# COMP6248-Reproducability-Challenge/selfsupervised-denoising

Hardware: AMD Instinct MI355X
Metric: training patches/sec (64x64 gauss25 SSDN) (higher is better)
Workload: dtype f16

## Files before the change

include/ssdn_hip.h:

```cpp
#ifndef SSDN_HIP_H
#define SSDN_HIP_H

#include <stdint.h>

#ifdef __cplusplus
extern "C" {
#endif
#if defined(__GNUC__) || defined(__clang__)
#pragma GCC visibility push(default)
#endif

#define SSDN_ABI_VERSION 19
#define SSDN_MAX_TAPS 9

typedef struct ssdn_view {
    void* p;
    int32_t cs;
    int32_t co;
} ssdn_view;

enum ssdn_op_type {
    SSDN_OP_PACK_INPUT = 1,
    SSDN_OP_CONV = 2,
    SSDN_OP_POOL_FWD = 3,
    SSDN_OP_POOL_BWD = 4,
    SSDN_OP_UPSUM_BWD = 5,
    SSDN_OP_UNROT_FWD = 6,
    SSDN_OP_UNROT_BWD = 7,
    SSDN_OP_WGRAD = 8,
    SSDN_OP_WREDUCE = 9,
    SSDN_OP_WPACK = 10,
    SSDN_OP_GRAD_PACK = 11,
    SSDN_OP_HEAD_SSDN = 12,
    SSDN_OP_HEAD_FINAL = 13,
    SSDN_OP_SPATIAL_MEAN = 14,
    SSDN_OP_MSE = 15,
    SSDN_OP_MASK_MSE = 16,
    SSDN_OP_ADAM = 17,
    SSDN_OP_METRICS = 18,
    SSDN_OP_ZERO = 19,
    SSDN_OP_EVENT_RECORD = 20,
    SSDN_OP_NOISE = 21,
    SSDN_OP_INPUT_GRAD = 22,
    SSDN_OP_HEAD_VJP = 23,
    SSDN_OP_MSE_VJP = 24,
    SSDN_OP_ACCUM = 25
};

typedef struct ssdn_op {
    int32_t type;
    int32_t lane;
    const void* args;
} ssdn_op;

typedef struct ssdn_pack_input_args {
    const float* src;
    ssdn_view dst;
    int32_t B, C, H, W;
    int32_t R;
    int32_t cpad;
} ssdn_pack_input_args;

typedef struct ssdn_conv_args {
    ssdn_view src0;
    ssdn_view src1;
    int32_t c0, c1, up0;
    int32_t N, H, W;
    int32_t ntaps;
    int32_t dy[SSDN_MAX_TAPS];
    int32_t dx[SSDN_MAX_TAPS];
    const void* w;
    int32_t M, Mpad, Ktot;
    const float* bias;
    int32_t act;
    ssdn_view mask;
    ssdn_view add;
    ssdn_view dst;
    float* dst32;
    int32_t ltw, lth, ltn;
    int32_t kc;
    int32_t bf16;
    const void* wc;
    int32_t kreal;
    ssdn_view pool;
    int32_t pool_shifted;
    ssdn_view upsum;
    ssdn_view upsum_mask;
    int32_t upsum_c;
    ssdn_view unrot;
    ssdn_view unrot_mask;
    const void* unrot_smask;
    ssdn_view urot;
    void* urot_smask;
    void* sign_out;
    const void* mask_sign;
    const void* upsum_mask_sign;
} ssdn_conv_args;

typedef struct ssdn_pool_args {
    ssdn_view act;
    ssdn_view pooled;
    ssdn_view dpool;
    ssdn_view dz;
    int32_t N, H, W, C;
    int32_t shifted;
    void* route;
} ssdn_pool_args;

typedef struct ssdn_upsum_args {
    ssdn_view src;
    ssdn_view mask;
    ssdn_view dst;
    int32_t N, H, W, C;
} ssdn_upsum_args;

typedef struct ssdn_unrot_args {
    ssdn_view src;
    ssdn_view dst;
    ssdn_view mask;
    int32_t B, P, C;
    void* smask;
} ssdn_unrot_args;

typedef struct ssdn_wgrad_args {
    ssdn_view dz;
    ssdn_view src0;
    ssdn_view src1;
    int32_t c0, c1, up0;
    int32_t N, H, W;
    int32_t ntaps;
    int32_t dy[SSDN_MAX_TAPS];
    int32_t dx[SSDN_MAX_TAPS];
    int32_t coff[SSDN_MAX_TAPS];
    int32_t M, Mpad, Ktot, Kpad;
    float* slab;
    float* bslab;
    int32_t nslabs;
    int32_t ltw, lth, ltn;
    int32_t csplit;
    int32_t mblocks;
    int32_t kreal;
    int32_t mega;
    float cost;
} ssdn_wgrad_args;

typedef struct ssdn_wreduce_args {
    const float* slab;
    const float* bslab;
    int32_t nslabs, ntaps, M, Mpad, Kpad;
    int32_t cin;
    int32_t cin_full;
    int32_t m_off, c_off;
    int32_t tapblock;
    float* gw;
    float* gb;
    const float* inv_scale;
    int32_t accumulate;
} ssdn_wreduce_args;

typedef struct ssdn_wpack_args {
    const float* w;
    void* wf;
    void* wd;
    int32_t M, cin, ntaps;
    int32_t c0, c1_real;
    int32_t Mpad_f, Ktot;
    int32_t Mpad_d, Kd;
    void* wfc;
    void* wdc;
} ssdn_wpack_args;

typedef struct ssdn_grad_pack_args {
    const float* g;
    ssdn_view dst;
    int32_t N, C, H, W, cpad;
    const uint32_t* gmax;
    float* scale_out;
} ssdn_grad_pack_args;

typedef struct ssdn_head_args {
    const float* net_out;
    const float* noisy;
    const float* noise_param;
    const float* est_raw;
    int32_t B, C, H, W;
    int32_t style, mode;
    int32_t want_grad;
    float* mu;
    float* pme;
    float* model_std;
    float* noise_std;
    float* g_net_out;
    float* partial;
    int32_t nchunks;
    uint32_t* gmax;
    int32_t diag;
} ssdn_head_args;

typedef struct ssdn_head_final_args {
    const float* partial;
    int32_t B, nchunks, H, W;
    int32_t mode;
    float* loss;
    float* g_est;
    float* g_sigma_out;
    uint32_t* gmax2;
} ssdn_head_final_args;

typedef struct ssdn_spatial_mean_args {
    const float* src;
    float* dst;
    int32_t B, HW;
} ssdn_spatial_mean_args;

typedef struct ssdn_mse_args {
    const float* out;
    const float* ref;
    const int64_t* coords;
    int32_t ncoords;
    int32_t B, C, H, W;
    float* loss;
    float* g;
    uint32_t* gmax;
} ssdn_mse_args;

typedef struct ssdn_head_vjp_args {
    const float* net_out;
    const float* noisy;
    const float* noise_param;
    const float* est_raw;
    int32_t B, C, H, W;
    int32_t style, mode;
    const float* w;
    const float* g_pme;
    const float* g_mu;
    int32_t keep;
    int32_t nchunks;
    float* g_net_out;
    float* partial;
    uint32_t* gmax;
    float* g_est;
    float* g_sigma_out;
    uint32_t* gmax2;
    float* g_noisy;
    int32_t diag;
} ssdn_head_vjp_args;

typedef struct ssdn_mse_vjp_args {
    const float* out;
    const float* ref;
    const int64_t* coords;
    int32_t ncoords;
    int32_t masked;
    int32_t B, C, H, W;
    int32_t keep;
    const float* w;
    const float* g_pme;
    float* g;
    uint32_t* gmax;
} ssdn_mse_vjp_args;

typedef struct ssdn_adam_args {
    float* p;
    const float* g;
    float* m;
    float* v;
    int64_t n;
    float lr, b1, b2, eps, bc1, bc2;
    float gscale;
} ssdn_adam_args;

typedef struct ssdn_metrics_args {
    const float* out;
    const float* mu;
    const float* clean;
    const float* loss;
    const float* model_std;
    const float* noise_std;
    const int32_t* ext;
    int32_t B, C, H, W;
    int32_t noise_n;
    float* per;
    float* acc;
} ssdn_metrics_args;

typedef struct ssdn_zero_args {
    void* p;
    int64_t bytes;
} ssdn_zero_args;

typedef struct ssdn_accum_args {
    float* dst;
    const float* src;
    int64_t n;
} ssdn_accum_args;

typedef struct ssdn_event_args {
    void* event;
} ssdn_event_args;

typedef struct ssdn_noise_args {
    const void* clean_u8;
    float* clean32;
    float* noisy32;
    float* ref32;
    float* param;
    float* param_ref;
    int64_t* coords;
    int32_t B, C, H, W;
    int32_t style;
    int32_t clip;
    float p_lo, p_hi;
    int32_t n2v_box;
    int32_t n2v_radius;
    uint64_t seed, offset;
} ssdn_noise_args;

typedef struct ssdn_input_grad_args {
    ssdn_view g_e0;
    ssdn_view g_d1a;
    const float* w_e;
    const float* w_d;
    float* out;
    int32_t B, C, H, W;
    int32_t R;
    int32_t ntaps;
    int32_t dy[SSDN_MAX_TAPS], dx[SSDN_MAX_TAPS];
    const float* add;
} ssdn_input_grad_args;

int ssdn_run_ops(const ssdn_op* ops, int n, void* stream);

int ssdn_stream_order(void* first, void* then);

int ssdn_conv_lds_bytes(const ssdn_conv_args* a);
int ssdn_wgrad_lds_bytes(const ssdn_wgrad_args* a);
int ssdn_wgrad_mega_ok(const ssdn_wgrad_args* a);
int ssdn_wgrad_variant(const ssdn_wgrad_args* a, int32_t* out9);

int ssdn_struct_size(int op_type);
int ssdn_abi_version(void);
const char* ssdn_last_error(void);
int ssdn_device_cus(void);

#define SSDN_PROF_CONV_MT3 0
#define SSDN_PROF_CONV_MT2 1
#define SSDN_PROF_CONV_MT1 2
#define SSDN_PROF_WGRAD 3
#define SSDN_PROF_GEMM 4
#define SSDN_PROF_CDMA_MT3 5
#define SSDN_PROF_CDMA_MT21 6
#define SSDN_PROF_WGRAD_SIDE 7
#define SSDN_PROF_KINDS 8
int ssdn_profile_enable(int kind, int max_launches);
int ssdn_profile_set_stride(int kind, int stride);
int ssdn_profile_read(int kind, double* total_ms, long long* launches, double* flops, double* bytes);

int ssdn_conv_set_mode(int mode);
int ssdn_conv_fuses_pool(const ssdn_conv_args* a);
int ssdn_conv_fuses_upsum(const ssdn_conv_args* a);
int ssdn_conv_fuses_unrot(const ssdn_conv_args* a);
int ssdn_conv_fuses_urot(const ssdn_conv_args* a);
int ssdn_conv_signs(const ssdn_conv_args* a);

int ssdn_chain_len(const ssdn_op* ops, int n);
int ssdn_conv_set_chain(int on);

int ssdn_wgrad_mergeable(const ssdn_wgrad_args* a);

#define SSDN_PLAN_REPACK 0
#define SSDN_PLAN_FORWARD 1
#define SSDN_PLAN_BACKWARD 2
#define SSDN_PLAN_OPTIMISER 3
#define SSDN_PLAN_PHASES 4
typedef struct ssdn_plan ssdn_plan;
int ssdn_plan_load(const void* blob, int64_t nbytes, ssdn_plan** out);
void ssdn_plan_destroy(ssdn_plan* plan);
int64_t ssdn_plan_arena_bytes(const ssdn_plan* plan);
const char* ssdn_plan_meta(const ssdn_plan* plan);
int ssdn_plan_bind(ssdn_plan* plan, void* arena);
int ssdn_plan_tensor(const ssdn_plan* plan, const char* name, void** ptr, int64_t* bytes);
int ssdn_plan_run(ssdn_plan* plan, int phase, void* stream);
int ssdn_plan_set_lr(ssdn_plan* plan, float lr, int step, float gscale);
int ssdn_net_forward(ssdn_plan* plan, void* stream);
int ssdn_train_step(ssdn_plan* plan, float lr, int step, void* stream);

void ssdn_debug_set_trace(void* device_buffer);
void* ssdn_debug_get_trace(void);

int ssdn_probe_mfma(const void* a_frag, const void* b_frag, float* d_out, void* stream);
int ssdn_probe_tr16(const void* lds_image, int image_bytes, const int32_t* lane_addr, void* out, void* stream);

#if defined(__GNUC__) || defined(__clang__)
#pragma GCC visibility pop
#endif
#ifdef __cplusplus
}
#endif
#endif
```

selfsupervised-denoising_amd/csrc/api.hip:

```cpp
#include "common.h"
#include <cstdarg>
#include <cstdio>
#include <cstdlib>

static thread_local char g_err[512] = "";
thread_local hipEvent_t g_ssdn_stop_event = nullptr;
thread_local bool g_ssdn_stop_used = false;
thread_local hipEvent_t g_ssdn_prof_start = nullptr, g_ssdn_prof_stop = nullptr;
thread_local bool g_ssdn_prof_used = false;

int ssdn_set_error(const char* fmt, ...) {
    va_list ap;
    va_start(ap, fmt);
    vsnprintf(g_err, sizeof(g_err), fmt, ap);
    va_end(ap);
    return -1;
}

#include <vector>
struct ProfSlot {
    bool on = false;
    std::vector<hipEvent_t> ev;
    size_t used = 0;
    double flops = 0.0, bytes = 0.0;
    long long seen = 0;
    int stride = 1;
    bool armed = false;
    bool attached = false;
};
static bool prof_single_launch(int id) { return id == SSDN_PROF_CDMA_MT3 || id == SSDN_PROF_CDMA_MT21 || id == SSDN_PROF_GEMM; }
static ProfSlot g_prof[SSDN_PROF_KINDS];

void prof_begin(int id, hipStream_t s) {
    ProfSlot& p = g_prof[id];
    p.armed = false;
    if (!p.on) return;
    const bool pick = p.seen++ % p.stride == 0;
    if (!pick || p.used + 2 > p.ev.size()) return;
    p.armed = true;
    p.attached = prof_single_launch(id) && !g_ssdn_stop_event;
    if (p.attached) {
        g_ssdn_prof_start = p.ev[p.used];
        g_ssdn_prof_stop = p.ev[p.used + 1];
        g_ssdn_prof_used = false;
    } else (void)hipEventRecord(p.ev[p.used], s);
}
void prof_end(int id, hipStream_t s, double flops, double bytes) {
    ProfSlot& p = g_prof[id];
    if (!p.on || !p.armed) return;
    p.armed = false;
    if (p.attached) {
        const bool used = g_ssdn_prof_used;
        g_ssdn_prof_start = g_ssdn_prof_stop = nullptr;
        g_ssdn_prof_used = false;
        if (!used) return;
    } else (void)hipEventRecord(p.ev[p.used + 1], s);
    p.used += 2;
    p.flops += flops;
    p.bytes += bytes;
}

__global__ void k_zero(uint4* p, long long n16) {
    long long i = (long long)blockIdx.x * blockDim.x + threadIdx.x;
    for (; i < n16; i += (long long)gridDim.x * blockDim.x) p[i] = make_uint4(0, 0, 0, 0);
}

extern "C" {

int ssdn_abi_version(void) { return SSDN_ABI_VERSION; }
const char* ssdn_last_error(void) { return g_err; }

int ssdn_device_cus(void) {
    int dev = 0, cus = 0;
    if (hipGetDevice(&dev) != hipSuccess) return ssdn_set_error("hipGetDevice failed");
    if (hipDeviceGetAttribute(&cus, hipDeviceAttributeMultiprocessorCount, dev) != hipSuccess)
        return ssdn_set_error("hipDeviceGetAttribute failed");
    return cus;
}

int ssdn_struct_size(int op_type) {
    switch (op_type) {
        case 0: return (int)sizeof(ssdn_op);
        case SSDN_OP_PACK_INPUT: return (int)sizeof(ssdn_pack_input_args);
        case SSDN_OP_CONV: return (int)sizeof(ssdn_conv_args);
        case SSDN_OP_POOL_FWD: case SSDN_OP_POOL_BWD: return (int)sizeof(ssdn_pool_args);
        case SSDN_OP_UPSUM_BWD: return (int)sizeof(ssdn_upsum_args);
        case SSDN_OP_UNROT_FWD: case SSDN_OP_UNROT_BWD: return (int)sizeof(ssdn_unrot_args);
        case SSDN_OP_WGRAD: return (int)sizeof(ssdn_wgrad_args);
        case SSDN_OP_WREDUCE: return (int)sizeof(ssdn_wreduce_args);
        case SSDN_OP_WPACK: return (int)sizeof(ssdn_wpack_args);
        case SSDN_OP_GRAD_PACK: return (int)sizeof(ssdn_grad_pack_args);
        case SSDN_OP_HEAD_SSDN: return (int)sizeof(ssdn_head_args);
        case SSDN_OP_HEAD_FINAL: return (int)sizeof(ssdn_head_final_args);
        case SSDN_OP_SPATIAL_MEAN: return (int)sizeof(ssdn_spatial_mean_args);
        case SSDN_OP_MSE: case SSDN_OP_MASK_MSE: return (int)sizeof(ssdn_mse_args);
        case SSDN_OP_ADAM: return (int)sizeof(ssdn_adam_args);
        case SSDN_OP_METRICS: return (int)sizeof(ssdn_metrics_args);
        case SSDN_OP_ZERO: return (int)sizeof(ssdn_zero_args);
        case SSDN_OP_EVENT_RECORD: return (int)sizeof(ssdn_event_args);
        case SSDN_OP_NOISE: return (int)sizeof(ssdn_noise_args);
        case SSDN_OP_INPUT_GRAD: return (int)sizeof(ssdn_input_grad_args);
        case SSDN_OP_HEAD_VJP: return (int)sizeof(ssdn_head_vjp_args);
        case SSDN_OP_MSE_VJP: return (int)sizeof(ssdn_mse_vjp_args);
        case SSDN_OP_ACCUM: return (int)sizeof(ssdn_accum_args);
        default: return -1;
    }
}

int ssdn_profile_enable(int kind, int max_launches) {
    if (kind < 0 || kind >= SSDN_PROF_KINDS) return ssdn_set_error("profile: bad kernel kind %d", kind);
    ProfSlot& p = g_prof[kind];
    for (hipEvent_t e : p.ev) (void)hipEventDestroy(e);
    p.ev.clear();
    p.used = 0;
    p.flops = p.bytes = 0.0;
    p.on = max_launches > 0;
    p.seen = 0;
    p.armed = false;
    for (int i = 0; i < 2 * max_launches; ++i) {
        hipEvent_t e;
        if (hipEventCreate(&e) != hipSuccess) return ssdn_set_error("profile: hipEventCreate failed");
        p.ev.push_back(e);
    }
    return 0;
}

int ssdn_profile_set_stride(int kind, int stride) {
    if (kind < 0 || kind >= SSDN_PROF_KINDS) return ssdn_set_error("profile: bad kernel kind %d", kind);
    if (stride < 1) return ssdn_set_error("profile: stride must be >= 1");
    g_prof[kind].stride = stride;
    return 0;
}

int ssdn_profile_read(int kind, double* total_ms, long long* launches, double* flops, double* bytes) {
    if (kind < 0 || kind >= SSDN_PROF_KINDS) return ssdn_set_error("profile: bad kernel kind %d", kind);
    ProfSlot& p = g_prof[kind];
    double ms = 0.0;
    for (size_t i = 0; i + 1 < p.used; i += 2) {
        if (hipEventSynchronize(p.ev[i + 1]) != hipSuccess) return ssdn_set_error("profile: hipEventSynchronize failed");
        float t = 0.f;
        if (hipEventElapsedTime(&t, p.ev[i], p.ev[i + 1]) != hipSuccess) return ssdn_set_error("profile: hipEventElapsedTime failed");
        ms += t;
    }
    *total_ms = ms;
    *launches = (long long)(p.used / 2);
    *flops = p.flops;
    *bytes = p.bytes;
    p.used = 0;
    p.flops = p.bytes = 0.0;
    return 0;
}

int ssdn_conv_lds_bytes(const ssdn_conv_args* a) { return conv_lds_bytes(a); }
int ssdn_wgrad_lds_bytes(const ssdn_wgrad_args* a) { return wgrad_lds_bytes(a); }
int ssdn_wgrad_mergeable(const ssdn_wgrad_args* a) { return a && wgrad_mergeable(a) ? 1 : 0; }
int ssdn_wgrad_mega_ok(const ssdn_wgrad_args* a) { return wgrad_mega_ok(a); }
int ssdn_conv_fuses_pool(const ssdn_conv_args* a) { return a && conv_fuses_pool(a) ? 1 : 0; }
int ssdn_conv_fuses_upsum(const ssdn_conv_args* a) { return a && conv_fuses_upsum(a) ? 1 : 0; }
int ssdn_conv_fuses_unrot(const ssdn_conv_args* a) { return a && conv_fuses_unrot(a) ? 1 : 0; }
int ssdn_conv_fuses_urot(const ssdn_conv_args* a) { return a && conv_fuses_urot(a) ? 1 : 0; }
int ssdn_conv_signs(const ssdn_conv_args* a) { return a && conv_signs(a) ? 1 : 0; }

#define SSDN_NEVENTS 256
#define SSDN_NLANES 4
#define SSDN_MAX_DEVICES 16
struct LaneSet {
    hipStream_t side[SSDN_NLANES] = {nullptr, nullptr, nullptr, nullptr};
    hipEvent_t ev[SSDN_NEVENTS];
    int ev_next = 0;
    bool ready = false;
};
static LaneSet g_lanesets[SSDN_MAX_DEVICES];
static LaneSet* lanes_get() {
    int dev = 0;
    if (hipGetDevice(&dev) != hipSuccess || dev < 0 || dev >= SSDN_MAX_DEVICES) { ssdn_set_error("lanes: bad current device"); return nullptr; }
    LaneSet& L = g_lanesets[dev];
    if (L.ready) return &L;
    for (int l = 1; l < SSDN_NLANES; ++l)
        if (hipStreamCreateWithFlags(&L.side[l], hipStreamNonBlocking) != hipSuccess) { ssdn_set_error("lanes: hipStreamCreate failed"); return nullptr; }
    for (int i = 0; i < SSDN_NEVENTS; ++i)
        if (hipEventCreateWithFlags(&L.ev[i], hipEventDisableTiming) != hipSuccess) { ssdn_set_error("lanes: hipEventCreate failed"); return nullptr; }
    L.ready = true;
    return &L;
}
static const unsigned g_lane_deps[SSDN_NLANES] = {0u, 1u << 0, (1u << 0) | (1u << 1) | (1u << 3), 1u << 0};

int ssdn_stream_order(void* first, void* then) {
    LaneSet* LS = lanes_get();
    if (!LS) return -1;
    hipEvent_t e = LS->ev[LS->ev_next++ % SSDN_NEVENTS];
    SSDN_CHECK_HIP(hipEventRecord(e, (hipStream_t)first));
    SSDN_CHECK_HIP(hipStreamWaitEvent((hipStream_t)then, e, 0));
    return 0;
}

int ssdn_run_ops(const ssdn_op* ops, int n, void* stream) {
    hipStream_t lane_s[SSDN_NLANES] = {(hipStream_t)stream, nullptr, nullptr, nullptr};
    g_ssdn_stop_event = nullptr;
    bool dirty[SSDN_NLANES][SSDN_NLANES] = {}, used[SSDN_NLANES] = {true, false, false, false};
    for (int d = 1; d < SSDN_NLANES; ++d) dirty[0][d] = true;
    static const bool one_lane = ssdn_tuning_env("SSDN_ONE_LANE") != nullptr;
    LaneSet* LS = nullptr;
    hipEvent_t cover[SSDN_NLANES] = {nullptr, nullptr, nullptr, nullptr};
    bool covered[SSDN_NLANES] = {false, false, false, false};
    long long cover_at[SSDN_NLANES] = {0, 0, 0, 0};
    auto cover_live = [&](int l) { return covered[l] && (!LS || (long long)LS->ev_next - cover_at[l] < SSDN_NEVENTS - 1); };
    bool has_side = false;
    static const bool no_stop = ssdn_tuning_env("SSDN_NO_STOP_EVENTS") != nullptr;
    for (int i = 0; i < n && !one_lane; ++i) has_side = has_side || ops[i].lane > 0;
    if (has_side && !(LS = lanes_get())) return -1;
    for (int i = 0; i < n; ++i) {
        const void* p = ops[i].args;
        int rc = 0;
        if (!p) return ssdn_set_error("op %d: null args", i);
        int lane = one_lane ? 0 : ops[i].lane;
        if (lane < 0 || lane >= SSDN_NLANES) return ssdn_set_error("op %d: bad lane %d", i, lane);
        if (lane > 0) {
            if (!LS && !(LS = lanes_get())) return -1;
            for (int l = 1; l < SSDN_NLANES; ++l) lane_s[l] = LS->side[l];
            for (int src = 0; src < SSDN_NLANES; ++src) {
                if (ops[i].type == SSDN_OP_EVENT_RECORD) break;
                if (!((g_lane_deps[lane] >> src) & 1) || !dirty[src][lane]) continue;
                if (!cover_live(src)) {
                    cover_at[src] = LS->ev_next;
                    cover[src] = LS->ev[LS->ev_next++ % SSDN_NEVENTS];
                    SSDN_CHECK_HIP(hipEventRecord(cover[src], lane_s[src]));
                    covered[src] = true;
                }
                SSDN_CHECK_HIP(hipStreamWaitEvent(lane_s[lane], cover[src], 0));
                dirty[src][lane] = false;
            }
        }
        const bool is_mark = ops[i].type == SSDN_OP_EVENT_RECORD;
        if (!is_mark) {
            for (int d = 0; d < SSDN_NLANES; ++d) dirty[lane][d] = true;
            covered[lane] = false;
        }
        used[lane] = true;
        hipStream_t s = lane_s[lane];
        bool armed = false;
        long long armed_at = 0;
        auto arm = [&](int j) {
            if (!has_side || no_stop || j >= n) return;
            const int lj = one_lane ? 0 : ops[j].lane;
            if (lj == lane || lj < 0 || lj >= SSDN_NLANES || !((g_lane_deps[lj] >> lane) & 1)) return;
            armed_at = LS->ev_next;
            g_ssdn_stop_event = LS->ev[LS->ev_next++ % SSDN_NEVENTS];
            g_ssdn_stop_used = false;
            armed = true;
        };
        auto arm_last = [&](int j) {
            if (!has_side || no_stop || lane == 0 || armed) return;
            for (; j < n; ++j)
                if ((one_lane ? 0 : ops[j].lane) == lane && ops[j].type != SSDN_OP_EVENT_RECORD) return;
            armed_at = LS->ev_next;
            g_ssdn_stop_event = LS->ev[LS->ev_next++ % SSDN_NEVENTS];
            g_ssdn_stop_used = false;
            armed = true;
        };
        switch (ops[i].type) {
            case SSDN_OP_PACK_INPUT: {
                const bool next_conv = i + 1 < n && ops[i + 1].type == SSDN_OP_CONV && ops[i + 1].args && (one_lane ? 0 : ops[i + 1].lane) == lane;
                if (next_conv && chain_merging_on() && conv_pack_fusable((const ssdn_pack_input_args*)p, (const ssdn_conv_args*)ops[i + 1].args)) {
                    rc = launch_conv_thin((const ssdn_conv_args*)ops[i + 1].args, (const ssdn_pack_input_args*)p, s);
                    ++i;
                } else rc = launch_pack_input((const ssdn_pack_input_args*)p, s);
                break;
            }
            case SSDN_OP_CONV: {
                const int m = chain_len(ops + i, n - i, one_lane);
                if (m < 0) return -1;
                const bool pair = m <= 1 && i + 1 < n && ops[i + 1].type == SSDN_OP_CONV && ops[i + 1].args && (one_lane ? 0 : ops[i + 1].lane) == lane &&
                                  chain_merging_on() && conv_pair_fusable((const ssdn_conv_args*)p, (const ssdn_conv_args*)ops[i + 1].args);
                arm(i + (m > 1 ? m : (pair ? 2 : 1)));
                if (m > 1) { rc = launch_chain(ops + i, m, one_lane, s); i += m - 1; }
                else if (pair) { rc = launch_gemm_dma_with_next((const ssdn_conv_args*)p, (const ssdn_conv_args*)ops[i + 1].args, s); ++i; }
                else rc = launch_conv((const ssdn_conv_args*)p, s);
                break;
            }
            case SSDN_OP_POOL_FWD: rc = launch_pool_fwd((const ssdn_pool_args*)p, s); break;
            case SSDN_OP_POOL_BWD: arm(i + 1); rc = launch_pool_bwd((const ssdn_pool_args*)p, s); break;
            case SSDN_OP_UPSUM_BWD: arm(i + 1); rc = launch_upsum_bwd((const ssdn_upsum_args*)p, s); break;
            case SSDN_OP_UNROT_FWD: rc = launch_unrot_fwd((const ssdn_unrot_args*)p, s); break;
            case SSDN_OP_UNROT_BWD: arm(i + 1); rc = launch_unrot_bwd((const ssdn_unrot_args*)p, s); break;
            case SSDN_OP_WGRAD: {
                static const bool no_merge = ssdn_tuning_env("SSDN_NO_WGRAD_MERGE") != nullptr;
                {
                    const ssdn_wgrad_args* mg[WGRAD_MEGA_MAX];
                    int mm = 0;
                    while (!no_merge && mm < WGRAD_MEGA_MAX && i + mm < n && ops[i + mm].type == SSDN_OP_WGRAD && ops[i + mm].args &&
                           (one_lane ? 0 : ops[i + mm].lane) == lane && wgrad_mega_ok((const ssdn_wgrad_args*)ops[i + mm].args) &&
                           ((const ssdn_wgrad_args*)ops[i + mm].args)->mega == ((const ssdn_wgrad_args*)p)->mega)
                        mg[mm] = (const ssdn_wgrad_args*)ops[i + mm].args, ++mm;
                    if (mm > 1) { arm(i + mm); rc = launch_wgrad_mega(mg, mm, s); i += mm - 1; break; }
                }
                const ssdn_wgrad_args* items[WGRAD_MULTI_MAX];
                int m = 0;
                while (!no_merge && m < WGRAD_MULTI_MAX && i + m < n && ops[i + m].type == SSDN_OP_WGRAD && ops[i + m].args &&
                       (one_lane ? 0 : ops[i + m].lane) == lane && wgrad_mergeable((const ssdn_wgrad_args*)ops[i + m].args))
                    items[m] = (const ssdn_wgrad_args*)ops[i + m].args, ++m;
                if (m > 1) { rc = launch_wgrad_multi(items, m, s); i += m - 1; }
                else rc = launch_wgrad((const ssdn_wgrad_args*)p, s);
                break;
            }
            case SSDN_OP_WREDUCE: {
                const ssdn_wreduce_args* items[WREDUCE_MULTI_MAX];
                int m = 0;
                while (m < WREDUCE_MULTI_MAX && i + m < n && ops[i + m].type == SSDN_OP_WREDUCE && ops[i + m].args &&
                       (one_lane ? 0 : ops[i + m].lane) == lane)
                    items[m] = (const ssdn_wreduce_args*)ops[i + m].args, ++m;
                arm_last(i + m);
                rc = m > 1 ? launch_wreduce_multi(items, m, s) : launch_wreduce((const ssdn_wreduce_args*)p, s);
                i += m - 1;
                break;
            }
            case SSDN_OP_WPACK: {
                const ssdn_wpack_args* items[WPACK_MULTI_MAX];
                int m = 0;
                while (m < WPACK_MULTI_MAX && i + m < n && ops[i + m].type == SSDN_OP_WPACK && ops[i + m].args &&
                       (one_lane ? 0 : ops[i + m].lane) == lane)
                    items[m] = (const ssdn_wpack_args*)ops[i + m].args, ++m;
                rc = m > 1 ? launch_wpack_multi(items, m, s) : launch_wpack((const ssdn_wpack_args*)p, s);
                i += m - 1;
                break;
            }
            case SSDN_OP_GRAD_PACK: {
                const bool next_conv = i + 1 < n && ops[i + 1].type == SSDN_OP_CONV && ops[i + 1].args && (one_lane ? 0 : ops[i + 1].lane) == lane;
                if (next_conv && chain_merging_on() && conv_gradpack_fusable((const ssdn_grad_pack_args*)p, (const ssdn_conv_args*)ops[i + 1].args)) {
                    arm(i + 2);
                    rc = launch_gradpack_dgrad((const ssdn_grad_pack_args*)p, (const ssdn_conv_args*)ops[i + 1].args, s);
                    ++i;
                } else { arm(i + 1); rc = launch_grad_pack((const ssdn_grad_pack_args*)p, s); }
                break;
            }
            case SSDN_OP_HEAD_SSDN: rc = launch_head((const ssdn_head_args*)p, s); break;
            case SSDN_OP_HEAD_FINAL: rc = launch_head_final((const ssdn_head_final_args*)p, s); break;
            case SSDN_OP_SPATIAL_MEAN: rc = launch_spatial_mean((const ssdn_spatial_mean_args*)p, s); break;
            case SSDN_OP_MSE: rc = launch_mse((const ssdn_mse_args*)p, 0, s); break;
            case SSDN_OP_MASK_MSE: rc = launch_mse((const ssdn_mse_args*)p, 1, s); break;
            case SSDN_OP_ADAM: {
                const ssdn_wpack_args* items[ADAM_PACK_MAX];
                int m = 0;
                while (m < ADAM_PACK_MAX && i + 1 + m < n && ops[i + 1 + m].type == SSDN_OP_WPACK && ops[i + 1 + m].args &&
                       (one_lane ? 0 : ops[i + 1 + m].lane) == lane)
                    items[m] = (const ssdn_wpack_args*)ops[i + 1 + m].args, ++m;
                const bool whole_run = !(i + 1 + m < n && ops[i + 1 + m].type == SSDN_OP_WPACK);
                if (m > 0 && whole_run && adam_pack_fusable((const ssdn_adam_args*)p, items, m)) {
                    rc = launch_adam_pack((const ssdn_adam_args*)p, items, m, s);
                    i += m;
                } else rc = launch_adam((const ssdn_adam_args*)p, s);
                break;
            }
            case SSDN_OP_METRICS: rc = launch_metrics((const ssdn_metrics_args*)p, s); break;
            case SSDN_OP_NOISE: rc = launch_noise((const ssdn_noise_args*)p, s); break;
            case SSDN_OP_INPUT_GRAD: arm(i + 1); rc = launch_input_grad((const ssdn_input_grad_args*)p, s); break;
            case SSDN_OP_HEAD_VJP: rc = launch_head_vjp((const ssdn_head_vjp_args*)p, s); break;
            case SSDN_OP_MSE_VJP: rc = launch_mse_vjp((const ssdn_mse_vjp_args*)p, s); break;
            case SSDN_OP_ACCUM: rc = launch_accum((const ssdn_accum_args*)p, s); break;
            case SSDN_OP_ZERO: {
                const ssdn_zero_args* z = (const ssdn_zero_args*)p;
                if (z->bytes & 15) return ssdn_set_error("op %d: zero size must be a multiple of 16", i);
                long long n16 = z->bytes / 16;
                int g = (int)((n16 + 255) / 256);
                if (g > 2048) g = 2048;
                if (g > 0) hipLaunchKernelGGL(k_zero, dim3(g), dim3(256), 0, s, (uint4*)z->p, n16);
                break;
            }
            case SSDN_OP_EVENT_RECORD: {
                const ssdn_event_args* e = (const ssdn_event_args*)p;
                if (!e->event) return ssdn_set_error("op %d: null event", i);
                SSDN_CHECK_HIP(hipEventRecord((hipEvent_t)e->event, s));
                break;
            }
            default: return ssdn_set_error("op %d: unknown type %d", i, ops[i].type);
        }
        if (armed) {
            if (g_ssdn_stop_used && !rc) { cover[lane] = g_ssdn_stop_event; covered[lane] = true; cover_at[lane] = armed_at; }
            g_ssdn_stop_event = nullptr;
        }
        if (rc) {
            char tmp[400];
            snprintf(tmp, sizeof(tmp), "%s", g_err);
            return ssdn_set_error("op %d (type %d): %s", i, ops[i].type, tmp);
        }
    }
    for (int l = 1; l < SSDN_NLANES; ++l) {
        if (!used[l]) continue;
        if (!cover_live(l)) {
            cover[l] = LS->ev[LS->ev_next++ % SSDN_NEVENTS];
            SSDN_CHECK_HIP(hipEventRecord(cover[l], lane_s[l]));
        }
        SSDN_CHECK_HIP(hipStreamWaitEvent(lane_s[0], cover[l], 0));
    }
    hipError_t e = hipGetLastError();
    if (e != hipSuccess) return ssdn_set_error("launch error: %s", hipGetErrorString(e));
    return 0;
}

}

__global__ void k_probe_mfma(const half8* a, const half8* b, float* d) {
    f32x16 acc;
#pragma unroll
    for (int r = 0; r < 16; ++r) acc[r] = 0.f;
    acc = __builtin_amdgcn_mfma_f32_32x32x16_f16(a[threadIdx.x], b[threadIdx.x], acc, 0, 0, 0);
#pragma unroll
    for (int r = 0; r < 16; ++r) d[threadIdx.x * 16 + r] = acc[r];
}

typedef __attribute__((__vector_size__(4 * sizeof(__fp16)))) __fp16 p_fp16x4_t;
typedef __attribute__((address_space(3))) p_fp16x4_t p_lds_fp16x4;
__global__ void k_probe_tr16(const uint4* image, int n16, const int* lane_addr, half4* out) {
    extern __shared__ __attribute__((aligned(16))) char smem[];
    for (int i = threadIdx.x; i < n16; i += blockDim.x) reinterpret_cast<uint4*>(smem)[i] = image[i];
    __syncthreads();
    p_fp16x4_t r = __builtin_amdgcn_ds_read_tr16_b64_v4f16((p_lds_fp16x4*)(smem + lane_addr[threadIdx.x]));
    out[threadIdx.x] = __builtin_bit_cast(half4, r);
}

extern "C" {
int ssdn_probe_mfma(const void* a_frag, const void* b_frag, float* d_out, void* stream) {
    hipLaunchKernelGGL(k_probe_mfma, dim3(1), dim3(64), 0, (hipStream_t)stream, (const half8*)a_frag, (const half8*)b_frag, d_out);
    hipError_t e = hipGetLastError();
    return e == hipSuccess ? 0 : ssdn_set_error("probe_mfma: %s", hipGetErrorString(e));
}
int ssdn_probe_tr16(const void* lds_image, int image_bytes, const int32_t* lane_addr, void* out, void* stream) {
    if (image_bytes & 15 || image_bytes > 64 * 1024) return ssdn_set_error("probe_tr16: bad image size");
    hipLaunchKernelGGL(k_probe_tr16, dim3(1), dim3(64), image_bytes, (hipStream_t)stream, (const uint4*)lds_image,
                       image_bytes / 16, lane_addr, (half4*)out);
    hipError_t e = hipGetLastError();
    return e == hipSuccess ? 0 : ssdn_set_error("probe_tr16: %s", hipGetErrorString(e));
}
}
```

selfsupervised-denoising_amd/csrc/common.h:

```cpp
#pragma once
#include <hip/hip_runtime.h>
#include <hip/hip_ext.h>
#include <stdint.h>
#include "../../include/ssdn_hip.h"
#include <cstdlib>

#if defined(SSDN_TUNING)
static inline const char* ssdn_tuning_env(const char* name) { return std::getenv(name); }
#else
static inline const char* ssdn_tuning_env(const char*) { return nullptr; }
#endif

typedef _Float16 h16;
typedef _Float16 half8 __attribute__((ext_vector_type(8)));
typedef _Float16 half4 __attribute__((ext_vector_type(4)));
typedef _Float16 half2v __attribute__((ext_vector_type(2)));
typedef __bf16 bf16x8 __attribute__((ext_vector_type(8)));
typedef unsigned short u16x8 __attribute__((ext_vector_type(8)));
typedef unsigned short u16x4 __attribute__((ext_vector_type(4)));
typedef float f32x16 __attribute__((ext_vector_type(16)));
typedef float f32x4 __attribute__((ext_vector_type(4)));

#define LRELU_SLOPE 0.1f

int ssdn_set_error(const char* fmt, ...);
#define SSDN_CHECK_HIP(expr)                                                                 \
    do {                                                                                     \
        hipError_t _e = (expr);                                                              \
        if (_e != hipSuccess) return ssdn_set_error("%s failed: %s", #expr, hipGetErrorString(_e)); \
    } while (0)

static __device__ __forceinline__ float lrelu(float v) { return v > 0.f ? v : LRELU_SLOPE * v; }
static __device__ __forceinline__ float lrelu_grad(float act) { return act > 0.f ? 1.f : LRELU_SLOPE; }

static __device__ __forceinline__ half8 ld_h8(const h16* p) { return *reinterpret_cast<const half8*>(p); }
static __device__ __forceinline__ void st_h8(h16* p, half8 v) { *reinterpret_cast<half8*>(p) = v; }
static __device__ __forceinline__ half4 ld_h4(const h16* p) { return *reinterpret_cast<const half4*>(p); }
static __device__ __forceinline__ void st_h4(h16* p, half4 v) { *reinterpret_cast<half4*>(p) = v; }

static __device__ __forceinline__ unsigned short f2bf(float f) {
    return __builtin_bit_cast(unsigned short, (__bf16)f);
}
static __device__ __forceinline__ float bf2f(unsigned short b) { return __uint_as_float(((unsigned)b) << 16); }
typedef __attribute__((__vector_size__(2 * sizeof(unsigned)))) unsigned u32x2_t;
typedef __attribute__((__vector_size__(4 * sizeof(unsigned)))) unsigned u32x4_t;
typedef __attribute__((__vector_size__(2 * sizeof(float)))) float f32x2_t;
typedef __attribute__((__vector_size__(2 * sizeof(__bf16)))) __bf16 bf16x2_t;
typedef __attribute__((__vector_size__(2 * sizeof(_Float16)))) _Float16 f16x2_t;
static __device__ __forceinline__ unsigned pack_bf16x2(float lo, float hi) {
    f32x2_t f = {lo, hi};
    return __builtin_bit_cast(unsigned, __builtin_convertvector(f, bf16x2_t));
}
static __device__ __forceinline__ unsigned pack_f16x2(float lo, float hi) {
    f32x2_t f = {lo, hi};
    return __builtin_bit_cast(unsigned, __builtin_convertvector(f, f16x2_t));
}
static __device__ __forceinline__ float bf_lo(unsigned w) { return __uint_as_float(w << 16); }
static __device__ __forceinline__ float bf_hi(unsigned w) { return __uint_as_float(w & 0xffff0000u); }
static __device__ __forceinline__ float f16_lo(unsigned w) { return (float)__builtin_bit_cast(f16x2_t, w)[0]; }
static __device__ __forceinline__ float f16_hi(unsigned w) { return (float)__builtin_bit_cast(f16x2_t, w)[1]; }
#define SSDN_BUFFER_RSRC_FLAGS 0x00020000
static __device__ __forceinline__ u16x8 ld_b8(const unsigned short* p) { return *reinterpret_cast<const u16x8*>(p); }
static __device__ __forceinline__ void st_b8(unsigned short* p, u16x8 v) { *reinterpret_cast<u16x8*>(p) = v; }
static __device__ __forceinline__ u16x4 ld_b4(const unsigned short* p) { return *reinterpret_cast<const u16x4*>(p); }
static __device__ __forceinline__ void st_b4(unsigned short* p, u16x4 v) { *reinterpret_cast<u16x4*>(p) = v; }
static __device__ __forceinline__ u16x8 zero_b8() {
    u16x8 z;
#pragma unroll
    for (int i = 0; i < 8; ++i) z[i] = 0;
    return z;
}

static __device__ __forceinline__ half8 zero_h8() {
    half8 z;
#pragma unroll
    for (int i = 0; i < 8; ++i) z[i] = (h16)0.f;
    return z;
}

extern thread_local hipEvent_t g_ssdn_stop_event;
extern thread_local bool g_ssdn_stop_used;
extern thread_local hipEvent_t g_ssdn_prof_start, g_ssdn_prof_stop;
extern thread_local bool g_ssdn_prof_used;
#define SSDN_LAUNCH(kernel, grid, block, lds, stream, ...)                                                                       \
    do {                                                                                                                         \
        if (g_ssdn_stop_event) {                                                                                                 \
            hipExtLaunchKernelGGL(kernel, grid, block, lds, stream, nullptr, g_ssdn_stop_event, 0, __VA_ARGS__);                 \
            g_ssdn_stop_used = true;                                                                                             \
        } else if (g_ssdn_prof_start) {                                                                                          \
            hipExtLaunchKernelGGL(kernel, grid, block, lds, stream, g_ssdn_prof_start, g_ssdn_prof_stop, 0, __VA_ARGS__);        \
            g_ssdn_prof_start = nullptr;                                                                                         \
            g_ssdn_prof_used = true;                                                                                             \
        } else hipLaunchKernelGGL(kernel, grid, block, lds, stream, __VA_ARGS__);                                                \
    } while (0)

#define SSDN_MAX_DEVICES_ATTR 16
static inline int ssdn_current_device_slot() {
    int dev = 0;
    if (hipGetDevice(&dev) != hipSuccess || dev < 0) dev = 0;
    return dev % SSDN_MAX_DEVICES_ATTR;
}

void prof_begin(int kind, hipStream_t s);
void prof_end(int kind, hipStream_t s, double flops, double bytes);

int launch_conv(const ssdn_conv_args* a, hipStream_t s);
int launch_wgrad(const ssdn_wgrad_args* a, hipStream_t s);
bool wgrad_mergeable(const ssdn_wgrad_args* a);
int launch_wgrad_multi(const ssdn_wgrad_args* const* items, int n, hipStream_t s);
#define WGRAD_MEGA_MAX 64
int wgrad_mega_ok(const ssdn_wgrad_args* a);
int launch_wgrad_mega(const ssdn_wgrad_args* const* ops, int n, hipStream_t s);
int launch_pack_input(const ssdn_pack_input_args* a, hipStream_t s);
int launch_pool_fwd(const ssdn_pool_args* a, hipStream_t s);
int launch_pool_bwd(const ssdn_pool_args* a, hipStream_t s);
int launch_upsum_bwd(const ssdn_upsum_args* a, hipStream_t s);
int launch_unrot_fwd(const ssdn_unrot_args* a, hipStream_t s);
int launch_unrot_bwd(const ssdn_unrot_args* a, hipStream_t s);
int launch_wreduce(const ssdn_wreduce_args* a, hipStream_t s);
int launch_wpack(const ssdn_wpack_args* a, hipStream_t s);
#define WPACK_MULTI_MAX 24
int launch_wpack_multi(const ssdn_wpack_args* const* items, int n, hipStream_t s);
#define WREDUCE_MULTI_MAX 32
#define WGRAD_MULTI_MAX 32
int launch_wreduce_multi(const ssdn_wreduce_args* const* items, int n, hipStream_t s);
int launch_grad_pack(const ssdn_grad_pack_args* a, hipStream_t s);
int launch_head(const ssdn_head_args* a, hipStream_t s);
int launch_head_impulse(const ssdn_head_args* a, hipStream_t s);
int launch_head_final(const ssdn_head_final_args* a, hipStream_t s);
int launch_spatial_mean(const ssdn_spatial_mean_args* a, hipStream_t s);
int launch_mse(const ssdn_mse_args* a, int masked, hipStream_t s);
int launch_head_vjp(const ssdn_head_vjp_args* a, hipStream_t s);
int launch_head_vjp_impulse(const ssdn_head_vjp_args* a, hipStream_t s);
int launch_mse_vjp(const ssdn_mse_vjp_args* a, hipStream_t s);
int launch_adam(const ssdn_adam_args* a, hipStream_t s);
#define ADAM_PACK_MAX 24
int adam_pack_fusable(const ssdn_adam_args* a, const ssdn_wpack_args* const* items, int n);
int launch_adam_pack(const ssdn_adam_args* a, const ssdn_wpack_args* const* items, int n, hipStream_t s);
int launch_metrics(const ssdn_metrics_args* a, hipStream_t s);
int launch_accum(const ssdn_accum_args* a, hipStream_t s);
int launch_noise(const ssdn_noise_args* a, hipStream_t s);
int launch_input_grad(const ssdn_input_grad_args* a, hipStream_t s);
int conv_lds_bytes(const ssdn_conv_args* a);
int conv_validate(const ssdn_conv_args* a);
int chain_len(const ssdn_op* ops, int n, bool any_lane);
int launch_chain(const ssdn_op* ops, int n, bool any_lane, hipStream_t s);
bool chain_merging_on();
bool conv_dma_eligible(const ssdn_conv_args* a, bool any_size);
int conv_dma_lds_bytes(int mt);
bool conv_signs(const ssdn_conv_args* a);
bool gemm_dma_signs(const ssdn_conv_args* a);
bool conv_dma_signs(const ssdn_conv_args* a);
bool conv_fuses_urot(const ssdn_conv_args* a);
bool conv_fuses_unrot(const ssdn_conv_args* a);
bool conv_fuses_upsum(const ssdn_conv_args* a);
bool conv_fuses_pool(const ssdn_conv_args* a);
int launch_conv_dma(const ssdn_conv_args* a, hipStream_t s);
bool conv_thin_eligible(const ssdn_conv_args* a);
bool conv_thin_fuses_pack(const ssdn_pack_input_args* pk, const ssdn_conv_args* a);
int launch_conv_thin(const ssdn_conv_args* a, const ssdn_pack_input_args* pk, hipStream_t s);
bool conv_pack_fusable(const ssdn_pack_input_args* pk, const ssdn_conv_args* a);
bool gradpack_dgrad_fusable(const ssdn_grad_pack_args* gp, const ssdn_conv_args* a);
int launch_gradpack_dgrad(const ssdn_grad_pack_args* gp, const ssdn_conv_args* a, hipStream_t s);
bool conv_gradpack_fusable(const ssdn_grad_pack_args* gp, const ssdn_conv_args* a);
bool gemm_dma_eligible(const ssdn_conv_args* a);
int gemm_dma_lds_bytes(const ssdn_conv_args* a);
int launch_gemm_dma(const ssdn_conv_args* a, hipStream_t s);
bool gemm_dma_fuses_next(const ssdn_conv_args* a, const ssdn_conv_args* b);
int launch_gemm_dma_with_next(const ssdn_conv_args* a, const ssdn_conv_args* b, hipStream_t s);
bool conv_pair_fusable(const ssdn_conv_args* a, const ssdn_conv_args* b);
extern "C" int ssdn_device_cus(void);
int wgrad_lds_bytes(const ssdn_wgrad_args* a);
```

selfsupervised-denoising_amd/csrc/head.hip:

```cpp
#include "head_common.h"

static __device__ __forceinline__ void diag_sigma(int style, int mode, float npar, float est, float mu, float& sig, float& dsig_dmu,
                                                  float& dsig_dest) {
    if (style == 0) {
        sig = mode == 0 ? fmaxf(npar, 1e-3f) : est;
        dsig_dmu = 0.f;
        dsig_dest = 1.f;
    } else {
        float m = fmaxf(mu, 1e-3f);
        float f = mode == 0 ? 1.f / npar : est;
        sig = sqrtf(m * f);
        dsig_dmu = mu > 1e-3f ? 0.5f * f / sig : 0.f;
        dsig_dest = 0.5f * m / sig;
    }
}
static __device__ __forceinline__ float diag_pme_weights(float sx, float sn, float& ix, float& in, float& u, float& v) {
    const float e = 1e-6f;
    ix = 1.f / (sx + e);
    in = 1.f / (sn + e);
    const float rD = 1.f / (ix + in + e);
    u = ix * rD;
    v = in * rD;
    return rD;
}

template <bool DIAG>
__global__ void k_head(ssdn_head_args a) {
    __shared__ float sh[4];
    const int b = blockIdx.y;
    const long long HW = (long long)a.H * a.W;
    const int C = a.C;
    const int Cout = DIAG ? 2 * C : C + C * (C + 1) / 2;
    const float inv_total = 1.f / ((float)a.B * (float)HW);
    float est = 0.f, dest_draw = 0.f;
    if (a.mode != 0) {
        float raw = a.est_raw[a.mode == 2 ? b : 0];
        est = softplus_m4(raw);
        dest_draw = sigmoid_m4(raw);
    }
    const float npar = a.noise_param ? a.noise_param[b] : 0.f;
    float loss_acc = 0.f, gest_acc = 0.f, gabs = 0.f;
    const long long per = (HW + a.nchunks - 1) / a.nchunks;
    const long long p0 = (long long)blockIdx.x * per;
    const long long p1 = p0 + per < HW ? p0 + per : HW;
    const float* no = a.net_out + (long long)b * Cout * HW;
    const float* ny = a.noisy + (long long)b * C * HW;
    for (long long p = p0 + threadIdx.x; p < p1; p += HB) {
        if constexpr (DIAG) {
            float mu[3], av[3], sig[3], dsig_dmu[3], dsig_dest[3], sx[3], sn[3], rs[3], q[3];
            float prod = 1.f, quad = 0.f;
#pragma unroll
            for (int c = 0; c < 3; ++c) {
                mu[c] = no[c * HW + p];
                av[c] = no[(3 + c) * HW + p];
                diag_sigma(a.style, a.mode, npar, est, mu[c], sig[c], dsig_dmu[c], dsig_dest[c]);
                sx[c] = av[c] * av[c];
                sn[c] = sig[c] * sig[c];
                const float sy = sx[c] + sn[c], d = ny[c * HW + p] - mu[c];
                rs[c] = 1.f / sy;
                q[c] = d * rs[c];
                prod *= sy;
                quad += d * q[c];
            }
            float l = 0.5f * logf(fmaxf(prod, 0.f)) + 0.5f * quad;
            if (a.mode != 0) l -= 0.1f * (sig[0] + sig[1] + sig[2]) * (1.f / 3.f);
            loss_acc += l;
            long long o3 = (long long)b * 3 * HW + p;
            if (a.mu) { a.mu[o3] = mu[0]; a.mu[o3 + HW] = mu[1]; a.mu[o3 + 2 * HW] = mu[2]; }
            if (a.pme) {
#pragma unroll
                for (int c = 0; c < 3; ++c) {
                    float ix, in, u, v;
                    diag_pme_weights(sx[c], sn[c], ix, in, u, v);
                    a.pme[o3 + c * HW] = mu[c] * u + ny[c * HW + p] * v;
                }
            }
            if (a.model_std) a.model_std[(long long)b * HW + p] = cbrtf(fabsf(av[0] * av[1] * av[2]));
            if (a.noise_std && a.style == 1) a.noise_std[(long long)b * HW + p] = cbrtf(sig[0] * sig[1] * sig[2]);
            if (a.want_grad) {
                const float hd = prod > 0.f ? 0.5f : 0.f;
                const float reg = a.mode != 0 ? 0.1f / 3.f : 0.f;
                float gs = 0.f;
#pragma unroll
                for (int c = 0; c < 3; ++c) {
                    const float gsy = hd * rs[c] - 0.5f * q[c] * q[c];
                    const float ds = 2.f * sig[c] * gsy - reg;
                    const float gmu = (-q[c] + ds * dsig_dmu[c]) * inv_total;
                    const float ga = 2.f * av[c] * gsy * inv_total;
                    a.g_net_out[((long long)b * 6 + c) * HW + p] = gmu;
                    a.g_net_out[((long long)b * 6 + 3 + c) * HW + p] = ga;
                    gabs = fmaxf(gabs, fmaxf(fabsf(gmu), fabsf(ga)));
                    gs += ds * dsig_dest[c];
                }
                gest_acc += gs;
            }
        } else if (C == 1) {
            float mu = no[p], av = no[HW + p], y = ny[p];
            float sig, dsig_dmu = 0.f, dsig_dest = 0.f;
            if (a.style == 0) {
                sig = a.mode == 0 ? fmaxf(npar, 1e-3f) : est;
                dsig_dest = 1.f;
            } else {
                float m = fmaxf(mu, 1e-3f);
                float f = a.mode == 0 ? 1.f / npar : est;
                sig = sqrtf(m * f);
                dsig_dmu = mu > 1e-3f ? 0.5f * f / sig : 0.f;
                dsig_dest = 0.5f * m / sig;
            }
            float sx = av * av, sn = sig * sig, sy = sx + sn;
            float d = y - mu;
            float l = d * d / sy + logf(sy);
            if (a.mode != 0) l -= 0.1f * sig;
            loss_acc += l;
            if (a.mu) a.mu[(long long)b * HW + p] = mu;
            if (a.pme) a.pme[(long long)b * HW + p] = (y * sx + mu * sn) / sy;
            if (a.model_std) a.model_std[(long long)b * HW + p] = fabsf(av);
            if (a.noise_std && a.style == 1) a.noise_std[(long long)b * HW + p] = sig;
            if (a.want_grad) {
                float dsy = -d * d / (sy * sy) + 1.f / sy;
                float dsig = 2.f * sig * dsy - (a.mode != 0 ? 0.1f : 0.f);
                float gmu = (-2.f * d / sy + dsig * dsig_dmu) * inv_total;
                float ga = 2.f * av * dsy * inv_total;
                a.g_net_out[(long long)b * 2 * HW + p] = gmu;
                a.g_net_out[(long long)b * 2 * HW + HW + p] = ga;
                gabs = fmaxf(gabs, fmaxf(fabsf(gmu), fabsf(ga)));
                gest_acc += dsig * dsig_dest;
            }
        } else {
            float mu[3], A[6], y[3], sig[3], dsig_dmu[3], dsig_dest[3];
#pragma unroll
            for (int c = 0; c < 3; ++c) { mu[c] = no[c * HW + p]; y[c] = ny[c * HW + p]; }
#pragma unroll
            for (int c = 0; c < 6; ++c) A[c] = no[(3 + c) * HW + p];
#pragma unroll
            for (int c = 0; c < 3; ++c) {
                if (a.style == 0) {
                    sig[c] = a.mode == 0 ? fmaxf(npar, 1e-3f) : est;
                    dsig_dmu[c] = 0.f;
                    dsig_dest[c] = 1.f;
                } else {
                    float m = fmaxf(mu[c], 1e-3f);
                    float f = a.mode == 0 ? 1.f / npar : est;
                    sig[c] = sqrtf(m * f);
                    dsig_dmu[c] = mu[c] > 1e-3f ? 0.5f * f / sig[c] : 0.f;
                    dsig_dest[c] = 0.5f * m / sig[c];
                }
            }
            float x00 = A[0] * A[0] + A[1] * A[1] + A[2] * A[2];
            float x01 = A[1] * A[3] + A[2] * A[4];
            float x02 = A[2] * A[5];
            float x11 = A[3] * A[3] + A[4] * A[4];
            float x12 = A[4] * A[5];
            float x22 = A[5] * A[5];
            float n0 = sig[0] * sig[0], n1 = sig[1] * sig[1], n2 = sig[2] * sig[2];
            float s00 = x00 + n0, s01 = x01, s02 = x02, s11 = x11 + n1, s12 = x12, s22 = x22 + n2;
            float c00 = s11 * s22 - s12 * s12, c01 = s02 * s12 - s01 * s22, c02 = s01 * s12 - s02 * s11;
            float c11 = s00 * s22 - s02 * s02, c12 = s01 * s02 - s00 * s12, c22 = s00 * s11 - s01 * s01;
            float det = s00 * c00 + s01 * c01 + s02 * c02;
            float rdet = 1.f / det;
            float i00 = c00 * rdet, i01 = c01 * rdet, i02 = c02 * rdet, i11 = c11 * rdet, i12 = c12 * rdet, i22 = c22 * rdet;
            float d0 = y[0] - mu[0], d1 = y[1] - mu[1], d2 = y[2] - mu[2];
            float q0 = i00 * d0 + i01 * d1 + i02 * d2;
            float q1 = i01 * d0 + i11 * d1 + i12 * d2;
            float q2 = i02 * d0 + i12 * d1 + i22 * d2;
            float quad = d0 * q0 + d1 * q1 + d2 * q2;
            float detc = fmaxf(det, 0.f);
            float l = 0.5f * logf(detc) + 0.5f * quad;
            if (a.mode != 0) l -= 0.1f * (sig[0] + sig[1] + sig[2]) * (1.f / 3.f);
            loss_acc += l;
            long long o3 = (long long)b * 3 * HW + p;
            if (a.mu) { a.mu[o3] = mu[0]; a.mu[o3 + HW] = mu[1]; a.mu[o3 + 2 * HW] = mu[2]; }
            if (a.pme) {
                const float e = 1e-6f;
                float t00 = s00 + 2 * e, t11 = s11 + 2 * e, t22 = s22 + 2 * e;
                float k00 = t11 * t22 - s12 * s12, k01 = s02 * s12 - s01 * t22, k02 = s01 * s12 - s02 * t11;
                float k11 = t00 * t22 - s02 * s02, k12 = s01 * s02 - t00 * s12, k22 = t00 * t11 - s01 * s01;
                float rd = 1.f / (t00 * k00 + s01 * k01 + s02 * k02);
                float r0 = (k00 * d0 + k01 * d1 + k02 * d2) * rd;
                float r1 = (k01 * d0 + k11 * d1 + k12 * d2) * rd;
                float r2 = (k02 * d0 + k12 * d1 + k22 * d2) * rd;
                a.pme[o3] = mu[0] + (x00 + e) * r0 + x01 * r1 + x02 * r2;
                a.pme[o3 + HW] = mu[1] + x01 * r0 + (x11 + e) * r1 + x12 * r2;
                a.pme[o3 + 2 * HW] = mu[2] + x02 * r0 + x12 * r1 + (x22 + e) * r2;
            }
            if (a.model_std) a.model_std[(long long)b * HW + p] = cbrtf(fabsf(A[0] * A[3] * A[5]));
            if (a.noise_std && a.style == 1) a.noise_std[(long long)b * HW + p] = cbrtf(sig[0] * sig[1] * sig[2]);
            if (a.want_grad) {
                float hd = det > 0.f ? 0.5f : 0.f;
                float g00 = hd * i00 - 0.5f * q0 * q0, g01 = hd * i01 - 0.5f * q0 * q1, g02 = hd * i02 - 0.5f * q0 * q2;
                float g11 = hd * i11 - 0.5f * q1 * q1, g12 = hd * i12 - 0.5f * q1 * q2, g22 = hd * i22 - 0.5f * q2 * q2;
                float reg = a.mode != 0 ? 0.1f / 3.f : 0.f;
                float ds0 = 2.f * sig[0] * g00 - reg, ds1 = 2.f * sig[1] * g11 - reg, ds2 = 2.f * sig[2] * g22 - reg;
                float g[9];
                g[0] = -q0 + ds0 * dsig_dmu[0];
                g[1] = -q1 + ds1 * dsig_dmu[1];
                g[2] = -q2 + ds2 * dsig_dmu[2];
                g[3] = 2.f * (g00 * A[0]);
                g[4] = 2.f * (g00 * A[1] + g01 * A[3]);
                g[5] = 2.f * (g00 * A[2] + g01 * A[4] + g02 * A[5]);
                g[6] = 2.f * (g01 * A[1] + g11 * A[3]);
                g[7] = 2.f * (g01 * A[2] + g11 * A[4] + g12 * A[5]);
                g[8] = 2.f * (g02 * A[2] + g12 * A[4] + g22 * A[5]);
#pragma unroll
                for (int c = 0; c < 9; ++c) {
                    float v = g[c] * inv_total;
                    a.g_net_out[((long long)b * 9 + c) * HW + p] = v;
                    gabs = fmaxf(gabs, fabsf(v));
                }
                gest_acc += ds0 * dsig_dest[0] + ds1 * dsig_dest[1] + ds2 * dsig_dest[2];
            }
        }
    }
    float ls = block_sum(loss_acc, sh);
    float gs = block_sum(gest_acc, sh);
    if (threadIdx.x == 0) {
        float* pp = a.partial + ((long long)b * a.nchunks + blockIdx.x) * 2;
        pp[0] = ls;
        pp[1] = gs * dest_draw * inv_total;
    }
    if (a.want_grad && a.gmax) atomic_max_abs_block(a.gmax, gabs, sh);
    if (blockIdx.x == 0 && threadIdx.x == 0 && a.noise_std && a.style == 0)
        a.noise_std[b] = a.mode == 0 ? fmaxf(npar, 1e-3f) : est;
}
int launch_head(const ssdn_head_args* a, hipStream_t s) {
    if (a->diag && a->C != 1 && a->C != 3) return ssdn_set_error("head: diag needs C = 1 or 3");
    if (a->C != 1 && a->C != 3) return ssdn_set_error("head: C must be 1 or 3 (denoiser.py:199)");
    if (a->diag != 0 && a->diag != 1) return ssdn_set_error("head: diag must be 0 or 1");
    if (a->nchunks < 1) return ssdn_set_error("head: nchunks < 1");
    if (a->style == 2) return launch_head_impulse(a, s);
    if (a->diag && a->C == 3) hipLaunchKernelGGL(k_head<true>, dim3(a->nchunks, a->B), dim3(HB), 0, s, *a);
    else hipLaunchKernelGGL(k_head<false>, dim3(a->nchunks, a->B), dim3(HB), 0, s, *a);
    return 0;
}

__global__ void k_head_final(ssdn_head_final_args a) {
    int b = blockIdx.x * blockDim.x + threadIdx.x;
    long long HW = (long long)a.H * a.W;
    if (b < a.B) {
        float l = 0.f, g = 0.f;
        for (int c = 0; c < a.nchunks; ++c) {
            l += a.partial[((long long)b * a.nchunks + c) * 2];
            g += a.partial[((long long)b * a.nchunks + c) * 2 + 1];
        }
        a.loss[b] = l / (float)HW;
        if (a.mode == 2 && a.g_est) a.g_est[b] = g;
    }
    if (a.mode == 1 && a.g_est && b == 0) {
        float g = 0.f;
        for (int bb = 0; bb < a.B; ++bb)
            for (int c = 0; c < a.nchunks; ++c) g += a.partial[((long long)bb * a.nchunks + c) * 2 + 1];
        a.g_est[0] = g;
    }
}
__global__ void k_fill_sigma_grad(ssdn_head_final_args a) {
    long long idx = (long long)blockIdx.x * blockDim.x + threadIdx.x;
    long long HW = (long long)a.H * a.W;
    if (idx >= a.B * HW) return;
    int b = idx / HW;
    float v = a.g_est[b] / (float)HW;
    a.g_sigma_out[idx] = v;
    if ((idx % HW) == 0 && v != 0.f && a.gmax2) atomicMax(a.gmax2, __float_as_uint(fabsf(v)));
}
int launch_head_final(const ssdn_head_final_args* a, hipStream_t s) {
    hipLaunchKernelGGL(k_head_final, dim3((a->B + 63) / 64), dim3(64), 0, s, *a);
    if (a->mode == 2 && a->g_sigma_out) {
        long long n = (long long)a->B * a->H * a->W;
        hipLaunchKernelGGL(k_fill_sigma_grad, dim3((int)((n + 255) / 256)), dim3(256), 0, s, *a);
    }
    return 0;
}

__global__ void k_spatial_mean(ssdn_spatial_mean_args a) {
    __shared__ float sh[4];
    int b = blockIdx.x;
    float acc = 0.f;
    for (int i = threadIdx.x; i < a.HW; i += HB) acc += a.src[(long long)b * a.HW + i];
    float t = block_sum(acc, sh);
    if (threadIdx.x == 0) a.dst[b] = t / (float)a.HW;
}
int launch_spatial_mean(const ssdn_spatial_mean_args* a, hipStream_t s) {
    hipLaunchKernelGGL(k_spatial_mean, dim3(a->B), dim3(HB), 0, s, *a);
    return 0;
}

__global__ void k_mse(ssdn_mse_args a) {
    __shared__ float sh[4];
    int b = blockIdx.x;
    long long n = (long long)a.C * a.H * a.W;
    float acc = 0.f, gabs = 0.f;
    float k = 2.f / ((float)n * (float)a.B);
    for (long long i = threadIdx.x; i < n; i += HB) {
        float d = a.out[b * n + i] - a.ref[b * n + i];
        acc += d * d;
        if (a.g) {
            float g = k * d;
            a.g[b * n + i] = g;
            gabs = fmaxf(gabs, fabsf(g));
        }
    }
    float t = block_sum(acc, sh);
    if (threadIdx.x == 0) a.loss[b] = t / (float)n;
    if (a.g && a.gmax) atomic_max_abs(a.gmax, gabs);
}
__global__ void k_mask_mse_zero(ssdn_mse_args a) {
    long long n = (long long)a.B * a.C * a.H * a.W;
    for (long long i = (long long)blockIdx.x * blockDim.x + threadIdx.x; i < n; i += (long long)gridDim.x * blockDim.x) a.g[i] = 0.f;
}
__global__ void k_mask_mse(ssdn_mse_args a) {
    __shared__ float sh[4];
    int b = blockIdx.x;
    long long HW = (long long)a.H * a.W;
    float acc = 0.f;
    float k = 2.f / ((float)a.C * (float)a.B);
    for (int c = threadIdx.x; c < a.C; c += HB) {
        for (int q = 0; q < a.ncoords; ++q) {
            long long r = a.coords[2 * q], cc = a.coords[2 * q + 1];
            if (r < 0 || r >= a.H || cc < 0 || cc >= a.W) continue;
            long long off = ((long long)b * a.C + c) * HW + r * a.W + cc;
            float d = a.out[off] - a.ref[off];
            acc += d * d;
            if (a.g) a.g[off] += k * d;
        }
    }
    float t = block_sum(acc, sh);
    if (threadIdx.x == 0) a.loss[b] = t / (float)a.C;
    if (a.g && a.gmax) {
        float gabs = 0.f;
        for (int c = threadIdx.x; c < a.C; c += HB)
            for (int q = 0; q < a.ncoords; ++q) {
                long long r = a.coords[2 * q], cc = a.coords[2 * q + 1];
                if (r < 0 || r >= a.H || cc < 0 || cc >= a.W) continue;
                gabs = fmaxf(gabs, fabsf(a.g[((long long)b * a.C + c) * HW + r * a.W + cc]));
            }
        atomic_max_abs(a.gmax, gabs);
    }
}
int launch_mse(const ssdn_mse_args* a, int masked, hipStream_t s) {
    if (!masked) {
        hipLaunchKernelGGL(k_mse, dim3(a->B), dim3(HB), 0, s, *a);
    } else {
        if (a->g) hipLaunchKernelGGL(k_mask_mse_zero, dim3(256), dim3(256), 0, s, *a);
        hipLaunchKernelGGL(k_mask_mse, dim3(a->B), dim3(HB), 0, s, *a);
    }
    return 0;
}

#define MB 1024
static __device__ __forceinline__ void metrics_block_sum4(float (&v)[4], float (*sh)[4]) {
#pragma unroll
    for (int k = 0; k < 4; ++k)
#pragma unroll
        for (int o = 32; o > 0; o >>= 1) v[k] += __shfl_down(v[k], o, 64);
    const int w = threadIdx.x >> 6, l = threadIdx.x & 63;
    if (l == 0) {
#pragma unroll
        for (int k = 0; k < 4; ++k) sh[w][k] = v[k];
    }
    __syncthreads();
#pragma unroll
    for (int k = 0; k < 4; ++k) {
        float t = 0.f;
#pragma unroll
        for (int j = 0; j < MB / 64; ++j) t += sh[j][k];
        v[k] = t;
    }
}
__global__ __launch_bounds__(MB) void k_metrics(ssdn_metrics_args a) {
    __shared__ float sh[MB / 64][4];
    __shared__ int last;
    const int b = blockIdx.x;
    const int HW = a.H * a.W;
    const int e1 = a.ext ? a.ext[2 * b] : a.H, e2 = a.ext ? a.ext[2 * b + 1] : a.W;
    const bool crop = e1 < a.H || e2 < a.W;
    float so = 0.f, sm = 0.f, ss = 0.f, sn = 0.f;
    const long long base = (long long)b * a.C * HW;
    constexpr int UNR = 6;
    const int n = a.C * HW;
    for (int i0 = threadIdx.x; i0 < n; i0 += MB * UNR) {
        float c[UNR], o[UNR], m[UNR];
#pragma unroll
        for (int u = 0; u < UNR; ++u) {
            const int i = i0 + u * MB;
            bool ok = i < n;
            if (crop) {
                const int p = i % HW, y = p / a.W, x = p - y * a.W;
                ok = ok && y < e1 && x < e2;
            }
            c[u] = ok ? a.clean[base + i] : 0.f;
            o[u] = (ok && a.out) ? a.out[base + i] : c[u];
            m[u] = (ok && a.mu) ? a.mu[base + i] : c[u];
        }
#pragma unroll
        for (int u = 0; u < UNR; ++u) {
            const float d0 = o[u] - c[u], d1 = m[u] - c[u];
            so += d0 * d0;
            sm += d1 * d1;
        }
    }
    const bool npix = a.noise_std && a.noise_n == a.B * HW;
    for (int i0 = threadIdx.x; i0 < HW; i0 += MB * 4) {
        float v[4], w[4];
#pragma unroll
        for (int u = 0; u < 4; ++u) {
            const int i = i0 + u * MB;
            v[u] = (a.model_std && i < HW) ? a.model_std[(long long)b * HW + i] : 0.f;
            w[u] = (npix && i < HW) ? a.noise_std[(long long)b * HW + i] : 0.f;
        }
#pragma unroll
        for (int u = 0; u < 4; ++u) { ss += v[u]; sn += w[u]; }
    }
    float sums[4] = {so, sm, ss, sn};
    metrics_block_sum4(sums, sh);
    so = sums[0]; sm = sums[1]; ss = sums[2]; sn = sums[3];
    if (threadIdx.x == 0) {
        const float cnt = (float)a.C * (float)e1 * (float)e2;
        float* q = a.per + 8 * b;
        q[0] = a.loss ? a.loss[b] : 0.f;
        q[1] = a.out ? -10.f * log10f(so / cnt) : 0.f;
        q[2] = a.mu ? -10.f * log10f(sm / cnt) : 0.f;
        q[3] = !a.noise_std ? 0.f : 255.f * (npix ? sn / (float)HW : a.noise_std[a.noise_n == a.B ? b : 0]);
        q[4] = a.model_std ? 255.f * ss / (float)HW : 0.f;
        __threadfence();
        const unsigned t = atomicAdd(reinterpret_cast<unsigned*>(a.acc + 15), 1u);
        last = t == (unsigned)a.B - 1;
    }
    __syncthreads();
    if (last && threadIdx.x < 64) {
        __threadfence();
        const int l = threadIdx.x;
        float v[5] = {0.f, 0.f, 0.f, 0.f, 0.f};
        for (int j = l; j < a.B; j += 64) {
            float q[5];
#pragma unroll
            for (int k = 0; k < 5; ++k) q[k] = __hip_atomic_load(a.per + 8 * j + k, __ATOMIC_RELAXED, __HIP_MEMORY_SCOPE_AGENT);
#pragma unroll
            for (int k = 0; k < 5; ++k) v[k] += q[k];
        }
        const float first3 = __hip_atomic_load(a.per + 3, __ATOMIC_RELAXED, __HIP_MEMORY_SCOPE_AGENT);
#pragma unroll
        for (int k = 0; k < 5; ++k)
#pragma unroll
            for (int off = 32; off > 0; off >>= 1) v[k] += __shfl_down(v[k], off);
        if (l == 0) {
#pragma unroll
            for (int k = 0; k < 5; ++k) {
                const bool on = k == 0 ? a.loss != nullptr : k == 1 ? a.out != nullptr : k == 2 ? a.mu != nullptr : k == 3 ? a.noise_std != nullptr : a.model_std != nullptr;
                if (!on) continue;
                const bool once = k == 3 && a.noise_n == 1;
                a.acc[2 * k] += once ? first3 : v[k];
                a.acc[2 * k + 1] += once ? 1.f : (float)a.B;
            }
            *reinterpret_cast<unsigned*>(a.acc + 15) = 0u;
        }
    }
}
int launch_metrics(const ssdn_metrics_args* a, hipStream_t s) {
    if (!a->clean || !a->per || !a->acc) return ssdn_set_error("metrics: clean, per and acc must be given");
    if (a->B < 1 || a->C < 1 || a->H < 1 || a->W < 1) return ssdn_set_error("metrics: bad shape");
    if (a->noise_std && a->noise_n != 1 && a->noise_n != a->B && a->noise_n != a->B * a->H * a->W) return ssdn_set_error("metrics: noise_n must be 1, B or B*H*W");
    hipLaunchKernelGGL(k_metrics, dim3(a->B), dim3(MB), 0, s, *a);
    return 0;
}

static __device__ __forceinline__ void head_dy_pixel(const ssdn_head_vjp_args& a, const float* no, const float* ny, const float* gp, float* gy,
                                                     long long p, long long HW, float sc, float npar, float est) {
    if (a.C == 1) {
        float mu = no[p], av = no[HW + p], y = ny[p];
        float sig;
        if (a.style == 0) sig = a.mode == 0 ? fmaxf(npar, 1e-3f) : est;
        else sig = sqrtf(fmaxf(mu, 1e-3f) * (a.mode == 0 ? 1.f / npar : est));
        float sx = av * av, sy = sx + sig * sig, rs = 1.f / sy, d = y - mu;
        float v = sc != 0.f ? 2.f * d * rs * sc : 0.f;
        if (gp) v += gp[p] * sx * rs;
        gy[p] = v;
        return;
    }
    float A[6], mu[3], n[3];
#pragma unroll
    for (int c = 0; c < 6; ++c) A[c] = no[(3 + c) * HW + p];
#pragma unroll
    for (int c = 0; c < 3; ++c) {
        mu[c] = no[c * HW + p];
        float sig;
        if (a.style == 0) sig = a.mode == 0 ? fmaxf(npar, 1e-3f) : est;
        else sig = sqrtf(fmaxf(mu[c], 1e-3f) * (a.mode == 0 ? 1.f / npar : est));
        n[c] = sig * sig;
    }
    float x00 = A[0] * A[0] + A[1] * A[1] + A[2] * A[2];
    float x01 = A[1] * A[3] + A[2] * A[4];
    float x02 = A[2] * A[5];
    float x11 = A[3] * A[3] + A[4] * A[4];
    float x12 = A[4] * A[5];
    float x22 = A[5] * A[5];
    float s00 = x00 + n[0], s11 = x11 + n[1], s22 = x22 + n[2];
    float d0 = ny[p] - mu[0], d1 = ny[HW + p] - mu[1], d2 = ny[2 * HW + p] - mu[2];
    float v0 = 0.f, v1 = 0.f, v2 = 0.f;
    if (sc != 0.f) {
        float c00 = s11 * s22 - x12 * x12, c01 = x02 * x12 - x01 * s22, c02 = x01 * x12 - x02 * s11;
        float c11 = s00 * s22 - x02 * x02, c12 = x01 * x02 - s00 * x12, c22 = s00 * s11 - x01 * x01;
        float rdet = 1.f / (s00 * c00 + x01 * c01 + x02 * c02);
        v0 = (c00 * d0 + c01 * d1 + c02 * d2) * rdet * sc;
        v1 = (c01 * d0 + c11 * d1 + c12 * d2) * rdet * sc;
        v2 = (c02 * d0 + c12 * d1 + c22 * d2) * rdet * sc;
    }
    if (gp) {
        const float e = 1e-6f;
        float ga0 = gp[p], ga1 = gp[HW + p], ga2 = gp[2 * HW + p];
        float t00 = s00 + 2 * e, t11 = s11 + 2 * e, t22 = s22 + 2 * e;
        float k00 = t11 * t22 - x12 * x12, k01 = x02 * x12 - x01 * t22, k02 = x01 * x12 - x02 * t11;
        float k11 = t00 * t22 - x02 * x02, k12 = x01 * x02 - t00 * x12, k22 = t00 * t11 - x01 * x01;
        float rd = 1.f / (t00 * k00 + x01 * k01 + x02 * k02);
        float u0 = (x00 + e) * ga0 + x01 * ga1 + x02 * ga2;
        float u1 = x01 * ga0 + (x11 + e) * ga1 + x12 * ga2;
// ... 332 lines not shown
```

selfsupervised-denoising_amd/csrc/head_common.h:

```cpp
#pragma once
#include "common.h"

#define HB 256

static __device__ __forceinline__ float block_sum(float v, float* sh) {
#pragma unroll
    for (int o = 32; o > 0; o >>= 1) v += __shfl_down(v, o, 64);
    int w = threadIdx.x >> 6, l = threadIdx.x & 63;
    __syncthreads();
    if (l == 0) sh[w] = v;
    __syncthreads();
    return sh[0] + sh[1] + sh[2] + sh[3];
}
static __device__ __forceinline__ void atomic_max_abs(uint32_t* gmax, float v) {
    float a = fabsf(v);
#pragma unroll
    for (int o = 32; o > 0; o >>= 1) a = fmaxf(a, __shfl_down(a, o, 64));
    if ((threadIdx.x & 63) == 0 && a > 0.f) atomicMax(gmax, __float_as_uint(a));
}
static __device__ __forceinline__ void atomic_max_abs_block(uint32_t* gmax, float v, float* sh4) {
    float a = fabsf(v);
#pragma unroll
    for (int o = 32; o > 0; o >>= 1) a = fmaxf(a, __shfl_down(a, o, 64));
    __syncthreads();
    if ((threadIdx.x & 63) == 0) sh4[threadIdx.x >> 6] = a;
    __syncthreads();
    if (threadIdx.x == 0) {
        const float m = fmaxf(fmaxf(sh4[0], sh4[1]), fmaxf(sh4[2], sh4[3]));
        if (m > 0.f) atomicMax(gmax, __float_as_uint(m));
    }
}
static __device__ __forceinline__ float softplus_m4(float raw) {
    float x = raw - 4.f;
    return (x > 20.f ? x : log1pf(expf(x))) + 1e-3f;
}
static __device__ __forceinline__ float sigmoid_m4(float raw) {
    float x = raw - 4.f;
    return x > 20.f ? 1.f : 1.f / (1.f + expf(-x));
}
```

selfsupervised-denoising_amd/ssdn/hip/engine.py:

```python
from __future__ import annotations

import os
import ctypes as C
import math
from typing import Dict, List, Optional

import torch

from . import lib as L
from .graph import NetPlan, Op, View


def _ptr(t: torch.Tensor, byte_off: int = 0) -> int:
    return t.data_ptr() + byte_off


class OpList:

    LANE = {"wgrad": (1,), "wreduce": (1,)}

    def __init__(self, recs, lanes: bool = False):
        self.args = [r[1] for r in recs]
        self.arr = (L.OpRec * max(1, len(recs)))()
        count = {}
        for i, r in enumerate(recs):
            ty, a = r[0], r[1]
            self.arr[i].type = L.OP[ty]
            choices = self.LANE.get(ty, (0,)) if lanes else (0,)
            self.arr[i].lane = choices[count.get(ty, 0) % len(choices)]
            if lanes and len(r) > 2:
                self.arr[i].lane = r[2]
            count[ty] = count.get(ty, 0) + 1
            self.arr[i].args = C.cast(C.pointer(a), C.c_void_p)
        self.n = len(recs)

    def run(self, stream: int = 0):
        if self.n:
            L.check(L.load().ssdn_run_ops(self.arr, self.n, C.c_void_p(stream)))


def current_stream() -> int:
    return torch.cuda.current_stream().cuda_stream


class DeviceNet:

    DT = {"act": torch.float16, "actb": torch.bfloat16, "f16": torch.float16, "bf16": torch.bfloat16, "f32": torch.float32,
          "u32": torch.int32, "i64": torch.int64, "u8": torch.uint8}

    def __init__(self, plan: NetPlan, device, params: torch.Tensor, grads: Optional[torch.Tensor],
                 shared: Optional[Dict[str, torch.Tensor]] = None, hold_input_grad: bool = False):
        self.plan, self.device = plan, device
        self.params, self.grads = params, grads
        self.t: Dict[str, torch.Tensor] = dict(shared or {})
        for name, spec in plan.tensors.items():
            if name in self.t:
                continue
            self.t[name] = torch.zeros(spec.shape, dtype=self.DT[spec.kind], device=device)
        self.fwd = OpList([self._mat(op) for op in plan.fwd])
        self._bwd_recs, self._bwd_layers = self._group_reductions(plan, [self._mat(op) for op in plan.bwd])
        k = next((i for i, r in enumerate(self._bwd_recs) if r[0] == "input_grad"), None)
        self.input_grad_args = self._bwd_recs[k][1] if k is not None else None
        self.input_grad_ops = None
        if hold_input_grad and k is not None:
            self.input_grad_ops = OpList([self._bwd_recs[k][:2]])
            del self._bwd_recs[k]
            del self._bwd_layers[k]
        self.bwd = OpList(self._bwd_recs, lanes=True)
        ntail = 0
        while ntail < len(self._bwd_recs) and self._bwd_recs[len(self._bwd_recs) - 1 - ntail][0] == "wreduce":
            ntail += 1
        self.tail_recs = [(r[0], r[1]) for r in self._bwd_recs[len(self._bwd_recs) - ntail:]] if 0 < ntail < len(self._bwd_recs) else []
        self.bwd_head = OpList(self._bwd_recs[:len(self._bwd_recs) - len(self.tail_recs)], lanes=True) if self.tail_recs else None
        self.pack = OpList([self._mat(op) for op in plan.pack])
        self.accumulate = False

    def set_accumulate(self, on: bool) -> None:
        self.accumulate = bool(on)
        for r in self._bwd_recs:
            if r[0] == "wreduce":
                r[1].accumulate = int(self.accumulate)

    def bwd_with_events(self, buckets, new_event):
        lane_of = lambda r: r[2] if len(r) > 2 else OpList.LANE.get(r[0], (0,))[0]
        last = {}
        for i, name in enumerate(self._bwd_layers):
            if name is None:
                continue
            for k, b in enumerate(buckets):
                if name in b:
                    last[(k, lane_of(self._bwd_recs[i]))] = i
        marks = {}
        for (k, lane), i in last.items():
            while i + 1 < len(self._bwd_recs) and self._bwd_recs[i + 1][0] == "wreduce" and lane_of(self._bwd_recs[i + 1]) == lane:
                i += 1
            marks.setdefault((i, lane), []).append(k)
        recs, self.marks = [], []
        for i, r in enumerate(self._bwd_recs):
            recs.append(r)
            for (idx, lane), ks in sorted(marks.items()):
                if idx == i:
                    recs.append(("event_record", L.EventArgs(new_event(sorted(ks))), lane))
                    self.marks.append((len(recs) - 1, lane, sorted(ks)))
        ol = OpList(recs, lanes=True)
        done_at = {}
        for (idx, lane), ks in marks.items():
            for k in ks:
                done_at[k] = max(done_at.get(k, -1), idx)
        by_pos = {}
        for k, idx in done_at.items():
            by_pos.setdefault(idx, []).append(k)
        ol.coincident = [sorted(ks) for _, ks in sorted(by_pos.items())]
        ol.marks = list(self.marks)
        return ol

    @staticmethod
    def _order_mega(plan, recs):
        side = lambda op: op.type in ("wgrad", "wreduce")
        gof = lambda op: plan.wgrad_group_of(op.a["layer"], plan.is_skip_half(op))
        flush = {}
        for i, op in enumerate(plan.bwd):
            if op.type == "wgrad":
                flush[gof(op)] = i
        lane_of = {}
        for g in list(flush):
            _, lane, after = plan.wgrad_group_info(g)
            lane_of[g] = MEGA_LANE if lane is None else lane
            if after is not None:
                at = [i for i, op in enumerate(plan.bwd) if op.type == "conv" and op.a["role"] == "dgrad" and op.a["layer"] == after]
                if at:
                    flush[g] = max(flush[g], at[0])
        def chainable(op):
            if op.type == "conv":
                px = op.a["H"] * op.a["W"]
                thin = px == 256 and op.a["Mpad"] <= 64 and op.a["Ktot"] <= 48 and op.a.get("upsum") is None
                return op.a["role"] == "dgrad" and len(op.a["taps"]) == 9 and (px <= 64 or thin)
            return op.type == "pool_bwd" and (op.a["H"] // 2) * (op.a["W"] // 2) <= 256
        windows, cur = [], None
        for i, op in enumerate(plan.bwd):
            if chainable(op):
                cur = [i, i] if cur is None else [cur[0], i]
            elif not side(op) and cur is not None:
                windows.append(cur)
                cur = None
        if cur is not None:
            windows.append(cur)
        for first, end in windows:
            for g in flush:
                if first <= flush[g] < end:
                    flush[g] = end
        out, names = [], []
        for i, (op, rec) in enumerate(zip(plan.bwd, recs)):
            if not side(op):
                out.append(rec)
                names.append(None)
            for g in sorted(flush):
                if flush[g] != i:
                    continue
                for op2, rec2 in zip(plan.bwd, recs):
                    if op2.type == "wgrad" and gof(op2) == g:
                        out.append((rec2[0], rec2[1], lane_of[g]))
                        names.append(None)
                for op2, rec2 in zip(plan.bwd, recs):
                    if op2.type == "wreduce" and gof(op2) == g:
                        out.append((rec2[0], rec2[1], lane_of[g]))
                        names.append(op2.a["layer"])
        return out, names

    @staticmethod
    def _group_reductions(plan, recs):
        if getattr(plan, "_mega_ops", None):
            return DeviceNet._order_mega(plan, recs)
        return DeviceNet._group_reductions_lanes(plan, recs)

    @staticmethod
    def _group_reductions_lanes(plan, recs):
        from .dp import bucket_layers
        if not plan.bwd:
            return recs, [op.a.get("layer") if op.type == "wreduce" else None for op in plan.bwd]
        buckets = bucket_layers(plan.layers, split_head=False)
        bucket_of = {name: k for k, b in enumerate(buckets) for name in b}
        from .graph import WGRAD_SMALL_PX
        small = lambda op: op.type == "wgrad" and op.a["N"] * op.a["H"] * op.a["W"] <= WGRAD_SMALL_PX
        flush_at = {}
        for i, op in enumerate(plan.bwd):
            if small(op):
                flush_at[bucket_of[op.a["layer"]]] = i
        nsmall = {k: sum(1 for op in plan.bwd if small(op) and bucket_of[op.a["layer"]] == k) for k in flush_at}
        flush_at = {k: i for k, i in flush_at.items() if nsmall[k] > 1}
        grouped = lambda op: small(op) and bucket_of[op.a["layer"]] in flush_at
        last = {}
        for i, op in enumerate(plan.bwd):
            if op.type in ("wgrad", "wreduce"):
                k = bucket_of[op.a["layer"]]
                last[k] = max(last.get(k, -1), flush_at[k] if grouped(op) else i)
        def chainable(op):
            if op.type == "conv":
                px = op.a["H"] * op.a["W"]
                thin = px == 256 and op.a["Mpad"] <= 64 and op.a["Ktot"] <= 48 and op.a.get("upsum") is None
                return op.a["role"] == "dgrad" and len(op.a["taps"]) == 9 and (px <= 64 or thin)
            return op.type == "pool_bwd" and (op.a["H"] // 2) * (op.a["W"] // 2) <= 256
        windows, cur = [], None
        for i, op in enumerate(plan.bwd):
            if chainable(op):
                cur = [i, i] if cur is None else [cur[0], i]
            elif op.type not in ("wgrad", "wreduce") and cur is not None:
                windows.append(cur)
                cur = None
        if cur is not None:
            windows.append(cur)
        for first, end in windows:
            for d in (flush_at, last):
                for k in d:
                    if first <= d[k] < end and (CHAIN_POSTPONES is None or k in CHAIN_POSTPONES):
                        d[k] = end
        out, names, pending = [], [], {k: [] for k in range(len(buckets))}
        pending_small = {k: [] for k in range(len(buckets))}
        pending_main = {k: [] for k in range(len(buckets))}
        hold_to, held = -1, []
        if plan.bwd[0].type == "grad_pack":
            j = next((k for k in range(1, len(plan.bwd)) if plan.bwd[k].type not in ("wgrad", "wreduce")), -1)
            if j > 1 and plan.bwd[j].type == "conv" and plan.bwd[j].a["role"] == "dgrad" and len(plan.bwd[j].a["taps"]) == 1 and plan.bwd[j].a["Ktot"] == 16:
                hold_to = j
        for i, (op, rec) in enumerate(zip(plan.bwd, recs)):
            if op.type == "wreduce":
                pending[bucket_of[op.a["layer"]]].append((rec, op.a["layer"]))
            elif op.type == "wgrad" and op.a["layer"] in MAIN_LANE_WGRADS:
                pending_main[bucket_of[op.a["layer"]]].append((rec[0], rec[1], 0))
            elif grouped(op):
                pending_small[bucket_of[op.a["layer"]]].append(rec)
            elif op.type == "wgrad" and i < hold_to:
                held.append(rec)
            else:
                out.append(rec)
                names.append(None)
                if i == hold_to:
                    out += held
                    names += [None] * len(held)
                    held = []
            for k in sorted(set(flush_at) | set(last)):
                if flush_at.get(k) == i:
                    out += pending_small[k]
                    names += [None] * len(pending_small[k])
                    pending_small[k] = []
                if not SPLIT_SMALL_RUNS:
                    continue
                if last.get(k) == i:
                    out += pending_main[k]
                    names += [None] * len(pending_main[k])
                    pending_main[k] = []
                    for rec_k, name_k in pending[k]:
                        out.append(rec_k)
                        names.append(name_k)
                    pending[k] = []
            for k in sorted(last):
                if last[k] == i and not SPLIT_SMALL_RUNS:
                    out += pending_main[k]
                    names += [None] * len(pending_main[k])
                    pending_main[k] = []
                    for rec_k, name_k in pending[k]:
                        out.append(rec_k)
                        names.append(name_k)
                    pending[k] = []
        return out, names

    def tensor(self, short: str) -> torch.Tensor:
        return self.t[self.plan.prefix + short]

    def _view(self, v: Optional[View]) -> L.View:
        if v is None:
            return L.View(None, 0, 0)
        t = self.t[v.t]
        return L.View(_ptr(t), t.shape[-1], v.co)

    def _pp(self, off_floats: int) -> int:
        return _ptr(self.params, 4 * (self.plan.param_base + off_floats))

    def _gp(self, off_floats: int) -> int:
        return _ptr(self.grads, 4 * (self.plan.param_base + off_floats))

    def _layer(self, name):
        return next(l for l in self.plan.layers if l.name == name)

    def _mat(self, op: Op):
        a = op.a
        P = self.plan.prefix
        if op.type == "pack_input":
            return op.type, L.PackInputArgs(_ptr(self.t[a["src"]]), self._view(a["dst"]), a["B"], a["C"], a["H"], a["W"], a["R"], a["cpad"])
        if op.type == "conv":
            l = self._layer(a["layer"])
            s = L.ConvArgs()
            s.src0, s.src1 = self._view(a["src0"]), self._view(a["src1"])
            s.c0, s.c1, s.up0 = a["c0"], a["c1"], a["up0"]
            s.N, s.H, s.W = a["N"], a["H"], a["W"]
            s.ntaps = len(a["taps"])
            for i, (dy, dx) in enumerate(a["taps"]):
                s.dy[i], s.dx[i] = dy, dx
            s.w = _ptr(self.t[P + ("wf/" if a["role"] == "fwd" else "wd/") + a["layer"]])
            wc = self.t.get(P + ("wfc/" if a["role"] == "fwd" else "wdc/") + a["layer"])
            s.wc = _ptr(wc) if wc is not None else None
            s.M, s.Mpad, s.Ktot = a["M"], a["Mpad"], a["Ktot"]
            s.bias = self._pp(l.b_off) if a["bias"] else None
            s.act = a["act"]
            s.mask, s.add, s.dst = self._view(a["mask"]), self._view(a["add"]), self._view(a["dst"])
            s.dst32 = _ptr(self.t[a["dst32"]]) if a["dst32"] is not None else None
            s.ltw, s.lth, s.ltn, s.kc = a["ltw"], a["lth"], a["ltn"], a["kc"]
            s.bf16 = a["bf16"]
            s.kreal = a.get("kreal", 0)
            s.pool, s.pool_shifted = self._view(a.get("pool")), a.get("pool_shifted", 0)
            if a.get("pool") is not None and not L.load().ssdn_conv_fuses_pool(C.byref(s)):
                raise L.SsdnHipError("conv %s: the plan fuses the max-pool but the library cannot (planner / library rule mismatch)" % a["layer"])
            s.upsum, s.upsum_mask, s.upsum_c = self._view(a.get("upsum")), self._view(a.get("upsum_mask")), a.get("upsum_c", 0)
            if a.get("upsum") is not None and not L.load().ssdn_conv_fuses_upsum(C.byref(s)):
                raise L.SsdnHipError("conv %s: the plan fuses UPSUM_BWD but the library cannot (planner / library rule mismatch)" % a["layer"])
            s.unrot, s.unrot_mask = self._view(a.get("unrot")), self._view(a.get("unrot_mask"))
            s.unrot_smask = self.t[a["unrot_smask"]].data_ptr() if a.get("unrot_smask") else None
            s.sign_out = self.t[a["sign_out"]].data_ptr() if a.get("sign_out") else None
            s.mask_sign = self.t[a["mask_sign"]].data_ptr() if a.get("mask_sign") else None
            s.upsum_mask_sign = self.t[a["upsum_mask_sign"]].data_ptr() if a.get("upsum_mask_sign") else None
            if (a.get("sign_out") or a.get("mask_sign") or a.get("upsum_mask_sign")) and not L.load().ssdn_conv_signs(C.byref(s)):
                raise L.SsdnHipError("conv %s: the plan uses sign bytes but the library cannot (planner / library rule mismatch)" % a["layer"])
            s.urot = self._view(a.get("urot"))
            s.urot_smask = self.t[a["urot_smask"]].data_ptr() if a.get("urot_smask") else None
            if a.get("urot") is not None and not L.load().ssdn_conv_fuses_urot(C.byref(s)):
                raise L.SsdnHipError("conv %s: the plan fuses UNROT_FWD but the library cannot (planner / library rule mismatch)" % a["layer"])
            if a.get("unrot") is not None and not L.load().ssdn_conv_fuses_unrot(C.byref(s)):
                raise L.SsdnHipError("conv %s: the plan fuses UNROT_BWD but the library cannot (planner / library rule mismatch)" % a["layer"])
            if L.load().ssdn_conv_lds_bytes(C.byref(s)) < 0:
                raise L.SsdnHipError("conv %s/%s: %s" % (a["layer"], a["role"], L.load().ssdn_last_error().decode()))
            return op.type, s
        if op.type in ("pool_fwd", "pool_bwd"):
            return op.type, L.PoolArgs(self._view(a["act"]), self._view(a.get("pooled")), self._view(a.get("dpool")),
                                       self._view(a.get("dz")), a["N"], a["H"], a["W"], a["C"], a["shifted"],
                                       self.t[a["route"]].data_ptr() if a.get("route") else None)
        if op.type == "upsum_bwd":
            return op.type, L.UpsumArgs(self._view(a["src"]), self._view(a["mask"]), self._view(a["dst"]), a["N"], a["H"], a["W"], a["C"])
        if op.type in ("unrot_fwd", "unrot_bwd"):
            return op.type, L.UnrotArgs(self._view(a["src"]), self._view(a["dst"]), self._view(a.get("mask")), a["B"], a["P"], a["C"],
                                        self.t[a["smask"]].data_ptr() if a.get("smask") else None)
        if op.type == "wgrad":
            s = L.WgradArgs()
            s.dz, s.src0, s.src1 = self._view(a["dz"]), self._view(a["src0"]), self._view(a["src1"])
            s.c0, s.c1, s.up0 = a["c0"], a["c1"], a["up0"]
            s.N, s.H, s.W = a["N"], a["H"], a["W"]
            s.ntaps = len(a["taps"])
            for i, (dy, dx) in enumerate(a["taps"]):
                s.dy[i], s.dx[i] = dy, dx
                s.coff[i] = a["coff"][i]
            s.M, s.Mpad, s.Ktot, s.Kpad = a["M"], a["Mpad"], a["Ktot"], a["Kpad"]
            s.slab, s.bslab = _ptr(self.t[a["slab"]]), _ptr(self.t[a["bslab"]])
            s.nslabs = a["nslabs"]
            s.ltw, s.lth, s.ltn = a["ltw"], a["lth"], a["ltn"]
            s.csplit = a.get("csplit", 0)
            s.mblocks = a.get("mblocks", 1)
            s.kreal = a.get("kreal", 0)
            s.mega, s.cost = a.get("mega", 0), a.get("cost", 0.0)
            if L.load().ssdn_wgrad_lds_bytes(C.byref(s)) < 0:
                raise L.SsdnHipError("wgrad %s: %s" % (a["layer"], L.load().ssdn_last_error().decode()))
            return op.type, s
        if op.type == "wreduce":
            l = self._layer(a["layer"])
            mb = a.get("mblock", 0)
            soff = 4 * mb * a["nslabs"] * a["ntaps"] * a["Mpad"] * a["Kpad"]
            boff = 4 * mb * a["nslabs"] * a["Mpad"]
            return op.type, L.WreduceArgs(_ptr(self.t[a["slab"]], soff), _ptr(self.t[a["bslab"]], boff), a["nslabs"], a["ntaps"], a["M"],
                                          a["Mpad"], a["Kpad"], a["cin"], a["cin_full"], a["m_off"], a["c_off"], a["tapblock"],
                                          self._gp(l.w_off), self._gp(l.b_off) if a["with_bias"] else None,
                                          _ptr(self.t[P + "scale"], 4))
        if op.type == "wpack":
            l = self._layer(a["layer"])
            return op.type, L.WpackArgs(self._pp(l.w_off), _ptr(self.t[P + "wf/" + l.name]),
                                        _ptr(self.t[P + "wd/" + l.name]) if a["need_d"] else None, a["M"], a["cin"], a["ntaps"],
                                        a["c0"], a["c1_real"], a["Mpad_f"], a["Ktot"], a["Mpad_d"], a["Kd"],
                                        _ptr(self.t[P + "wfc/" + l.name]) if a.get("cm_f") else None,
                                        _ptr(self.t[P + "wdc/" + l.name]) if a.get("cm_d") else None)
        if op.type == "grad_pack":
            return op.type, L.GradPackArgs(_ptr(self.t[a["g"]]), self._view(a["dst"]), a["N"], a["C"], a["H"], a["W"], a["cpad"],
                                           _ptr(self.t[P + "gmax"]), _ptr(self.t[P + "scale"]))
        if op.type == "input_grad":
            s = L.InputGradArgs()
            s.g_e0, s.g_d1a = self._view(a["g_e0"]), self._view(a["g_d1a"])
            s.w_e, s.w_d = self._pp(self._layer(a["layer_e"]).w_off), self._pp(self._layer(a["layer_d"]).w_off)
            s.out = _ptr(self.t[a["dst"]])
            s.B, s.C, s.H, s.W, s.R = a["B"], a["C"], a["H"], a["W"], a["R"]
            s.ntaps = len(a["taps"])
            for i, (dy, dx) in enumerate(a["taps"]):
                s.dy[i], s.dx[i] = dy, dx
            return op.type, s
        raise ValueError("unknown op type " + op.type)


MAIN_LANE_WGRADS = ("encode_block_1.0", "encode_block_1.2")
SPLIT_SMALL_RUNS = True
DEFER_TAIL = True
CHAIN_POSTPONES = (2,)

HEAD_PX_PER_BLOCK = 1024

MEGA_LANE = 0

STYLE = {"gauss": 0, "poisson": 1, "impulse": 2}
MODE = {"known": 0, "const": 1, "var": 2}


def engine_style(style: str) -> str:
    return "poisson" if style.startswith("poisson") else "impulse" if style.startswith("impulse") else "gauss"


class DenoiserEngine:

    def __init__(self, pipeline: str, channels: int, blindspot: bool, style: str, mode: str, B: int, H: int, W: int,
                 device, params: torch.Tensor, grads: torch.Tensor, adam_m: torch.Tensor, adam_v: torch.Tensor,
                 n_main: int, n_sigma: int, has_est: bool, train: bool = True, ncoords: int = 64, input_grad: bool = False,
                 diag: bool = False):
        if input_grad and not train:
            raise ValueError("input_grad needs a training engine (train=True)")
        self.pipeline, self.C, self.blindspot, self.mode = pipeline, channels, blindspot, mode
        self.diag = bool(diag) and pipeline == "ssdn"
        self.input_grad = bool(input_grad)
        self.style = engine_style(style)
        if self.style == "impulse" and self.diag:
            raise NotImplementedError("DIAGONAL_COVARIANCE is not implemented for the impulse noise model")
        self.B, self.H, self.W, self.device, self.train = B, H, W, device, train
        self.params, self.grads, self.m, self.v = params, grads, adam_m, adam_v
        lib = L.load()
        cus = lib.ssdn_device_cus()
        if cus <= 0:
            raise L.SsdnHipError("no HIP device: " + lib.ssdn_last_error().decode())
        cout = (2 * channels if self.diag else channels + channels * (channels + 1) // 2) if pipeline == "ssdn" else channels
        f32 = dict(dtype=torch.float32, device=device)
        self.inp = torch.zeros((B, channels, H, W), **f32)
        var = pipeline == "ssdn" and mode == "var"
        self.main = DeviceNet(NetPlan("m/", channels, cout, blindspot, B, H, W, cus=cus, train=train, param_base=0, input_grad=self.input_grad),
                              device, params, grads, shared={"m/in32": self.inp}, hold_input_grad=self.input_grad and var)
        self.sigma = None
        if var:
            self.sigma = DeviceNet(NetPlan("s/", channels, 1, False, B, H, W, cus=cus, train=train, param_base=n_main, input_grad=self.input_grad),
                                   device, params, grads, shared={"s/in32": self.inp})
        self.dx = None
        if self.input_grad:
            self.dx = self.main.tensor("dx32")
            if self.sigma is not None:
                self.main.input_grad_args.add = _ptr(self.sigma.tensor("dx32"))
        self.est_off = n_main + n_sigma if has_est else None
        self.loss = torch.zeros((B, 1), **f32)
        self.ref = torch.zeros((B, channels, H, W), **f32)
        self.noise_param = torch.zeros((B,), **f32)
        self.coords = torch.zeros((ncoords, 2), dtype=torch.int64, device=device)
        self.ncoords = ncoords
        self.nchunks = max(1, min(64, (H * W) // HEAD_PX_PER_BLOCK))
        self.partial = torch.zeros((B, self.nchunks, 2), **f32)
        self.est_raw = torch.zeros((B,), **f32)
        self.g_est_var = torch.zeros((B,), **f32)
        self.mu = torch.zeros((B, channels, H, W), **f32)
        self.pme = torch.zeros((B, channels, H, W), **f32)
        self.model_std = torch.zeros((B, H, W), **f32)
        self.noise_std = torch.zeros((B, H, W) if self.style == "poisson" else (B,), **f32)
        self.zero_buf = torch.zeros((8,), dtype=torch.int32, device=device)
        self._adam_args = None
        self.accumulate = False
        self.stages_est = bool(train and pipeline == "ssdn" and mode == "const" and self.est_off is not None)
        self.g_est_stage = torch.zeros((1,), **f32) if self.stages_est else None
        self._head_final_args = None
        self._accum_ops = None
        self.metrics_per = torch.zeros((B, 8), **f32)
        self._metrics_args = None
        self.ops_loss = OpList(self._loss_ops(want_grad=train))
        opt_recs = self._opt_ops() if train else None
        self.ops_opt = OpList(opt_recs) if train else None
        self.ops_opt_tail = OpList(self.main.tail_recs + opt_recs) if train and self.main.tail_recs else None
        self._tail_pending = False
        self.gen = 0
        self.g_fresh = self.loss_fwd = False
        self._vjp = None

    def _gmax(self, net: Optional[DeviceNet]):
        if net is not None and self.train:
            return _ptr(net.tensor("gmax"))
        return _ptr(self.zero_buf)

    def _loss_ops(self, want_grad: bool):
        recs = []
        B, Cn, H, W = self.B, self.C, self.H, self.W
        out32 = self.main.tensor("out32")
        g32 = _ptr(self.main.tensor("g32")) if want_grad else None
        if self.pipeline == "ssdn":
            est_ptr = None
            if self.mode == "var":
                recs.append(("spatial_mean", L.SpatialMeanArgs(_ptr(self.sigma.tensor("out32")), _ptr(self.est_raw), B, H * W)))
                est_ptr = _ptr(self.est_raw)
            elif self.mode == "const":
                est_ptr = _ptr(self.params, 4 * self.est_off)
            recs.append(("head_ssdn", L.HeadArgs(_ptr(out32), _ptr(self.inp), _ptr(self.noise_param), est_ptr, B, Cn, H, W,
                                                  STYLE[self.style], MODE[self.mode], int(want_grad), _ptr(self.mu), _ptr(self.pme),
                                                  _ptr(self.model_std), _ptr(self.noise_std), g32, _ptr(self.partial),
                                                  self.nchunks, self._gmax(self.main), int(self.diag))))
            g_est = self._g_est_ptr() if want_grad else None
            recs.append(("head_final", L.HeadFinalArgs(_ptr(self.partial), B, self.nchunks, H, W, MODE[self.mode], _ptr(self.loss), g_est,
                                                        _ptr(self.sigma.tensor("g32")) if (want_grad and self.sigma is not None) else None,
                                                        self._gmax(self.sigma) if self.sigma is not None else None)))
            self._head_final_args = recs[-1][1]
        elif self.pipeline == "mse":
            recs.append(("mse", L.MseArgs(_ptr(out32), _ptr(self.ref), None, 0, B, Cn, H, W, _ptr(self.loss), g32, self._gmax(self.main))))
        elif self.pipeline == "mask_mse":
            recs.append(("mask_mse", L.MseArgs(_ptr(out32), _ptr(self.ref), _ptr(self.coords), self.ncoords, B, Cn, H, W, _ptr(self.loss),
                                               g32, self._gmax(self.main))))
        else:
            raise NotImplementedError("Unsupported processing pipeline")
        return recs

    def _g_est_ptr(self):
        if self.mode == "const":
            return _ptr(self.g_est_stage) if self.accumulate and self.stages_est else _ptr(self.grads, 4 * self.est_off)
        if self.mode == "var":
            return _ptr(self.g_est_var)
        return None

    def set_accumulate(self, on: bool) -> None:
        on = bool(on)
        if on == self.accumulate:
            return
        if on and not self.train:
            raise L.SsdnHipError("set_accumulate needs a training engine")
        self.accumulate = on
        self.main.set_accumulate(on)
        if self.sigma is not None:
            self.sigma.set_accumulate(on)
        if self.stages_est:
            if self._head_final_args is not None and self._head_final_args.g_est:
                self._head_final_args.g_est = self._g_est_ptr()
            if self._vjp is not None:
                self._vjp[0].g_est = self._g_est_ptr()
            if on and self._accum_ops is None:
                self._accum_ops = OpList([("accum", L.AccumArgs(_ptr(self.grads, 4 * self.est_off), _ptr(self.g_est_stage), 1))])

    def _opt_ops(self):
        def adam(lo, hi):
            return L.AdamArgs(_ptr(self.params, 4 * lo), _ptr(self.grads, 4 * lo), _ptr(self.m, 4 * lo), _ptr(self.v, 4 * lo), hi - lo,
                              0.0, 0.9, 0.99, 1e-8, 1.0, 1.0, 1.0)
        n_tot = self.params.numel()
        n_main = self.sigma.plan.param_base if self.sigma is not None else n_tot
        self._adam_args = [adam(0, n_main)]
        recs = [("adam", self._adam_args[0])] + [self.main._mat(op) for op in self.main.plan.pack]
        if self.sigma is not None:
            self._adam_args.append(adam(n_main, n_tot))
            recs += [("adam", self._adam_args[1])] + [self.sigma._mat(op) for op in self.sigma.plan.pack]
        return recs

    def accumulate_metrics(self, acc: torch.Tensor, clean: torch.Tensor, ext: Optional[torch.Tensor] = None, with_loss: bool = True,
                           stream=None):
        a = self._metrics_args
        if a is None:
            a = self._metrics_args = L.MetricsArgs()
            a.B, a.C, a.H, a.W = self.B, self.C, self.H, self.W
            a.per = _ptr(self.metrics_per)
            if self.pipeline == "ssdn":
                a.out, a.mu, a.model_std, a.noise_std = _ptr(self.pme), _ptr(self.mu), _ptr(self.model_std), _ptr(self.noise_std)
                a.noise_n = self.noise_std.numel() if self.style == "poisson" else (1 if self.mode == "const" else self.B)
            else:
                a.out = _ptr(self.main.tensor("out32"))
            self._metrics_ops = OpList([("metrics", a)])
        if clean.dtype != torch.float32 or not clean.is_contiguous() or tuple(clean.shape) != (self.B, self.C, self.H, self.W):
            raise L.SsdnHipError("metrics: clean must be a contiguous fp32 [B,C,H,W] device tensor of the engine's shape")
        a.clean, a.acc = _ptr(clean), _ptr(acc)
        a.loss = _ptr(self.loss) if with_loss else None
        a.ext = _ptr(ext) if ext is not None else None
        self._metrics_ops.run(current_stream() if stream is None else stream)

    def export_plan(self, meta: Optional[dict] = None) -> bytes:
        if self.input_grad:
            raise L.SsdnHipError("export_plan: input-gradient engines (the autograd route's) are not part of the plan blob")
        if self.accumulate:
            self.set_accumulate(False)
            try:
                return self.export_plan(meta)
            finally:
                self.set_accumulate(True)
        import json
        import struct
        tens: List[tuple] = []
        for name, t in self.main.t.items():
            tens.append((name, t))
        if self.sigma is not None:
            for name, t in self.sigma.t.items():
                tens.append((name, t))
        tens += [("params", self.params), ("grads", self.grads), ("adam_m", self.m), ("adam_v", self.v), ("loss", self.loss), ("ref", self.ref),
                 ("noise_param", self.noise_param), ("coords", self.coords), ("partial", self.partial), ("est_raw", self.est_raw),
                 ("g_est_var", self.g_est_var), ("mu", self.mu), ("pme", self.pme), ("model_std", self.model_std), ("noise_std", self.noise_std),
                 ("zero_buf", self.zero_buf), ("metrics_per", self.metrics_per)]
        tens = [(n, t) for n, t in tens if t is not None]
        table, by_ptr = [], {}
        for name, t in tens:
            nbytes = t.numel() * t.element_size()
            ptr = t.data_ptr()
            alias = by_ptr.get(ptr, -1)
            if alias >= 0 and table[alias][1] < nbytes:
                raise L.SsdnHipError("export_plan: tensor %s aliases a smaller one" % name)
            if alias < 0:
                by_ptr[ptr] = len(table)
            table.append((name, nbytes, alias, ptr))
        spans = sorted((ptr, ptr + nb, i) for i, (n, nb, al, ptr) in enumerate(table) if al < 0)

        def locate(v):
            for lo, hi, i in spans:
                if lo <= v < hi or (v == hi == lo):
                    return i, v - lo
            raise L.SsdnHipError("export_plan: an op argument points outside every tensor of the engine (0x%x)" % v)
        ptr_off = {ty: L.pointer_fields(ty) for ty in set(L.ARG_TYPES.values())}

        def ser(oplists):
            out, n = b"", 0
            for ol in oplists:
                if ol is None:
                    continue
                for i in range(ol.n):
                    a = ol.args[i]
                    raw = bytes(a)
                    rel = b""
                    nr = 0
                    for off in ptr_off[type(a)]:
                        v = struct.unpack_from("<Q", raw, off)[0]
                        if v:
                            ti, d = locate(v)
                            rel += struct.pack("<IIQ", off, ti, d)
                            nr += 1
                    pad = (-len(raw)) % 8
                    out += struct.pack("<iiII", int(ol.arr[i].type), int(ol.arr[i].lane), len(raw), nr) + raw + b"\0" * pad + rel
                    n += 1
            return struct.pack("<I", n) + out
        train = self.train
        phases = [[self.main.pack, self.sigma.pack if self.sigma is not None else None],
                  [self.main.fwd, self.sigma.fwd if self.sigma is not None else None, self.ops_loss],
                  [self.main.bwd, self.sigma.bwd if self.sigma is not None else None] if train else [],
                  [self.ops_opt] if train else []]
        layers = lambda net, base: [dict(name=l.name, w_off=base + l.w_off, b_off=base + l.b_off, M=l.M, cin=l.cin, k=l.k) for l in net.plan.layers]
        desc = dict(pipeline=self.pipeline, channels=self.C, blindspot=bool(self.blindspot), style=self.style, mode=self.mode, diag=self.diag, B=self.B, H=self.H,
                    W=self.W, train=bool(train), nparams=int(self.params.numel()), est_off=self.est_off,
                    layers=layers(self.main, 0) + (layers(self.sigma, self.sigma.plan.param_base) if self.sigma is not None else []))
        desc.update(meta or {})
        mj = json.dumps(desc).encode()
        blob = b"SSDNPLAN" + struct.pack("<IIII", 1, L.ABI_VERSION, len(table), 4)
        for name, nb, al, _ in table:
            nm = name.encode()
            if len(nm) > 55:
                raise L.SsdnHipError("export_plan: tensor name too long: " + name)
            blob += nm + b"\0" * (56 - len(nm)) + struct.pack("<Qii", nb, al, 0)
        for ph in phases:
            blob += ser(ph)
        return blob + struct.pack("<I", len(mj)) + mj

    def repack(self, stream=None):
        s = current_stream() if stream is None else stream
        self.main.pack.run(s)
        if self.sigma is not None:
            self.sigma.pack.run(s)

    SIGMA_CONCURRENT = 3

    def _fork_sigma(self, s: int, oplist) -> int:
        if getattr(self, "_side", None) is None:
            self._side = torch.cuda.Stream(device=self.device)
        side = self._side.cuda_stream
        L.check(L.load().ssdn_stream_order(C.c_void_p(s), C.c_void_p(side)))
        oplist.run(side)
        return side

    def _join_sigma(self, s: int, side: int) -> None:
        L.check(L.load().ssdn_stream_order(C.c_void_p(side), C.c_void_p(s)))

    def forward(self, stream=None):
        s = current_stream() if stream is None else stream
        if self.train:
            self.gen += 1
            self.g_fresh = self.loss_fwd = True
        if self.sigma is not None and (int(self.SIGMA_CONCURRENT) & 1):
            ev = self._fork_sigma(s, self.sigma.fwd)
            self.main.fwd.run(s)
            self._join_sigma(s, ev)
        else:
            self.main.fwd.run(s)
            if self.sigma is not None:
                self.sigma.fwd.run(s)
        self.ops_loss.run(s)

    def net_forward_only(self, stream=None):
        s = current_stream() if stream is None else stream
        if self.train:
            self.gen += 1
            self.g_fresh = self.loss_fwd = False
        self.main.fwd.run(s)

    def _head_addend(self, on: bool) -> None:
        if not self.input_grad or self.pipeline != "ssdn":
            return
        first = self.sigma if self.sigma is not None else self.main
        first.input_grad_args.add = _ptr(self.dx) if on else None

    def backward(self, stream=None, exchange=None, defer_tail=False, with_head_dx=False):
        s = current_stream() if stream is None else stream
        self._head_addend(with_head_dx)
        if self.accumulate and self.stages_est:
            self._accum_ops.run(s)
        if defer_tail and exchange is None and self.ops_opt_tail is not None:
            if self.sigma is not None and (int(self.SIGMA_CONCURRENT) & 2):
                ev = self._fork_sigma(s, self.sigma.bwd)
                self.main.bwd_head.run(s)
                self._join_sigma(s, ev)
            else:
                self.main.bwd_head.run(s)
                if self.sigma is not None:
                    self.sigma.bwd.run(s)
            self._held_input_grad(s)
            self._tail_pending = True
            return
        self._tail_pending = False
        if exchange is not None and exchange.overlapped:
            from .dp import bucket_layers, N_MAIN_BUCKETS as NB
            if getattr(self, "_bwd_ev_key", None) != id(exchange):
                exchange.reset_marks()
                self._bwd_ev = self.main.bwd_with_events(bucket_layers(self.main.plan.layers), exchange.new_event)
                self._bwd_ev_key = id(exchange)
                if len(exchange.ranges) > NB:
                    exchange.record_here(NB)
                self._bwd_ev_marks = (exchange.events, exchange.waits, exchange._here)
                self._bwd_ev_groups = [list(g) for g in self._bwd_ev.coincident] + [[k] for k in range(NB, len(exchange.ranges))]
            exchange.events, exchange.waits, exchange._here = self._bwd_ev_marks
            exchange.groups = self._bwd_ev_groups
            self._bwd_ev.run(s)
            if self.sigma is not None:
                self.sigma.bwd.run(s)
            if len(exchange.ranges) > NB:
                exchange.record_here(NB)
            self._held_input_grad(s)
            return
        if self.sigma is not None and (int(self.SIGMA_CONCURRENT) & 2):
            ev = self._fork_sigma(s, self.sigma.bwd)
            self.main.bwd.run(s)
            self._join_sigma(s, ev)
        else:
            self.main.bwd.run(s)
            if self.sigma is not None:
                self.sigma.bwd.run(s)
        self._held_input_grad(s)

    def _held_input_grad(self, s: int) -> None:
        if self.main.input_grad_ops is not None:
            self.main.input_grad_ops.run(s)

    def _vjp_setup(self):
        f32 = dict(dtype=torch.float32, device=self.device)
        B, Cn, H, W = self.B, self.C, self.H, self.W
        self.vjp_w = torch.zeros((B,), **f32)
        self.vjp_g_pme = torch.zeros((B, Cn, H, W), **f32)
        self.vjp_g_mu = torch.zeros((B, Cn, H, W), **f32) if self.pipeline == "ssdn" else None
        g32 = _ptr(self.main.tensor("g32"))
        if self.pipeline == "ssdn":
            a = L.HeadVjpArgs()
            a.net_out, a.noisy, a.noise_param = _ptr(self.main.tensor("out32")), _ptr(self.inp), _ptr(self.noise_param)
            a.B, a.C, a.H, a.W, a.style, a.mode = B, Cn, H, W, STYLE[self.style], MODE[self.mode]
            a.nchunks, a.g_net_out, a.partial, a.gmax = self.nchunks, g32, _ptr(self.partial), self._gmax(self.main)
            a.diag = int(self.diag)
            if self.mode == "const":
                a.est_raw, a.g_est = _ptr(self.params, 4 * self.est_off), self._g_est_ptr()
            elif self.mode == "var":
                a.est_raw, a.g_est = _ptr(self.est_raw), _ptr(self.g_est_var)
                a.g_sigma_out, a.gmax2 = _ptr(self.sigma.tensor("g32")), self._gmax(self.sigma)
            self._vjp = (a, OpList([("head_vjp", a)]))
        else:
            a = L.MseVjpArgs(_ptr(self.main.tensor("out32")), _ptr(self.ref), _ptr(self.coords), self.ncoords, int(self.pipeline == "mask_mse"),
                             B, Cn, H, W, 0, None, None, g32, self._gmax(self.main))
            self._vjp = (a, OpList([("mse_vjp", a)]))

    def vjp_backward(self, w: Optional[torch.Tensor] = None, g_pme: Optional[torch.Tensor] = None, g_mu: Optional[torch.Tensor] = None,
                     stream=None, want_dx: bool = False):
        if not self.train:
            raise L.SsdnHipError("vjp_backward needs a training engine")
        if want_dx and not self.input_grad:
            raise L.SsdnHipError("vjp_backward(want_dx=True) needs an engine built with input_grad=True")
        if self._vjp is None:
            self._vjp_setup()
        a, ops = self._vjp
        a.w = a.g_pme = None
        if w is not None:
            self.vjp_w.copy_(w.reshape(self.B), non_blocking=True)
            a.w = _ptr(self.vjp_w)
        if g_pme is not None:
            self.vjp_g_pme.copy_(g_pme, non_blocking=True)
            a.g_pme = _ptr(self.vjp_g_pme)
        if self.pipeline == "ssdn":
            a.g_mu = None
            if g_mu is not None:
                self.vjp_g_mu.copy_(g_mu, non_blocking=True)
                a.g_mu = _ptr(self.vjp_g_mu)
            a.g_noisy = _ptr(self.dx) if want_dx else None
        elif g_mu is not None:
            raise L.SsdnHipError("the %s pipeline has no IMG_MU" % self.pipeline)
        a.keep = int(self.g_fresh)
        s = current_stream() if stream is None else stream
        ops.run(s)
        self.g_fresh = False
        self.backward(stream=s, with_head_dx=want_dx and self.pipeline == "ssdn")

    def adam(self, lr: float, step: int, gscale: float = 1.0, stream=None):
        for a in self._adam_args:
            a.lr, a.bc1, a.bc2, a.gscale = lr, 1.0 - 0.9 ** step, 1.0 - 0.99 ** step, gscale
        s = current_stream() if stream is None else stream
        if self._tail_pending:
            self._tail_pending = False
            self.ops_opt_tail.run(s)
            return
        self.ops_opt.run(s)
```

selfsupervised-denoising_amd/ssdn/hip/graph.py:

```python
from __future__ import annotations

import os
from dataclasses import dataclass, field
from typing import Dict, List, Optional, Tuple

LDS_LIMIT = 160 * 1024
CONV_LDS_PREFERRED = 80 * 1024
WGRAD_SMALL_PX = 32768
SMALL_WGRAD_G, SMALL_WGRAD_CUS = 2, 64
MID_WGRAD_PX, MID_WGRAD_G = 131072, 2
WGRAD_CU_FRAC = (3, 4)
WGRAD_MEGA = "split"
FUSE_UNROT_FWD = True
SIGN_BYTES_HEAD = True
X16_SLOTS = 16
POOL_ROUTE = True
SIGN_BYTES_CONV = True
SIGN_BYTES = True
MEGA_MIN_PX = 32768
SPLIT_HEAD_CUS = (1, 2)
SPLIT_AFTER = "decode_block_2.2"
SPLIT_GROUP0 = ("output_block", "decode_block_2.2")
MEGA_COST = {
    "static": (342.0, 38.8),
    "static2": (258.0, 40.2),
    "generic": (1350.0, 53.0),
    "head": (1208.0, 0.0),
    "head_mb": (1208.0, 0.0),
    "thin": (2211.0, 963.0),
    "sync_tile": 9000.0,
    "fixed": 30000.0,
    "slab_rate": 10.0,
}
TAPS_BLIND = [(ky - 2, kx - 1) for ky in range(3) for kx in range(3)]
TAPS_PLAIN = [(ky - 1, kx - 1) for ky in range(3) for kx in range(3)]
TAPS_1x1 = [(0, 0)]


def ceil_to(v: int, m: int) -> int:
    return (v + m - 1) // m * m


@dataclass
class TSpec:
    name: str
    kind: str
    shape: Tuple[int, ...]


@dataclass
class View:
    t: str
    co: int = 0


@dataclass
class Op:
    type: str
    a: dict = field(default_factory=dict)


@dataclass
class Layer:
    name: str
    M: int
    cin: int
    k: int
    c0: int
    c1: int
    c1_real: int
    w_off: int = 0
    b_off: int = 0

    @property
    def ntaps(self):
        return self.k * self.k

    @property
    def Ktot(self):
        return self.c0 + self.c1

    @property
    def Mpad_f(self):
        return ceil_to(self.M, 32)

    @property
    def Kd(self):
        return ceil_to(self.M, 16)


def net_layers(in_channels: int, out_channels: int, blindspot: bool) -> List[Layer]:
    c = in_channels
    cpad = 16
    nin = 384 if blindspot else 96
    L = [
        Layer("encode_block_1.0", 48, c, 3, cpad, 0, 0),
        Layer("encode_block_1.2", 48, 48, 3, 48, 0, 0),
        Layer("encode_block_2.0", 48, 48, 3, 48, 0, 0),
        Layer("encode_block_3.0", 48, 48, 3, 48, 0, 0),
        Layer("encode_block_4.0", 48, 48, 3, 48, 0, 0),
        Layer("encode_block_5.0", 48, 48, 3, 48, 0, 0),
        Layer("encode_block_6.0", 48, 48, 3, 48, 0, 0),
        Layer("decode_block_5.0", 96, 96, 3, 48, 48, 48),
        Layer("decode_block_5.2", 96, 96, 3, 96, 0, 0),
        Layer("decode_block_4.0", 96, 144, 3, 96, 48, 48),
        Layer("decode_block_4.2", 96, 96, 3, 96, 0, 0),
        Layer("decode_block_3.0", 96, 144, 3, 96, 48, 48),
        Layer("decode_block_3.2", 96, 96, 3, 96, 0, 0),
        Layer("decode_block_2.0", 96, 144, 3, 96, 48, 48),
        Layer("decode_block_2.2", 96, 96, 3, 96, 0, 0),
        Layer("decode_block_1.0", 96, 96 + c, 3, 96, cpad, c),
        Layer("decode_block_1.2", 96, 96, 3, 96, 0, 0),
        Layer("output_block.0", nin, nin, 1, nin, 0, 0),
        Layer("output_block.2", 96, nin, 1, nin, 0, 0),
        Layer("output_block.4", out_channels, 96, 1, 96, 0, 0),
    ]
    L[0].c0, L[0].c1, L[0].c1_real = 0, cpad, c
    off = 0
    for l in L:
        l.w_off = off
        off += l.M * l.cin * l.k * l.k
        l.b_off = off
        off += l.M
    return L


def net_param_count(layers: List[Layer]) -> int:
    return layers[-1].b_off + layers[-1].M



def _pads(taps):
    dys = [t[0] for t in taps]
    dxs = [t[1] for t in taps]
    return max(0, -min(dys)), max(0, max(dys)), max(0, -min(dxs)), max(0, max(dxs))


def _pow2ceil_log(v: int) -> int:
    l = 0
    while (1 << l) < v:
        l += 1
    return l


def cdma_fills(tiles: int, cus: int, H: int = 0, W: int = 0) -> bool:
    return tiles >= cus or (2 * tiles >= cus and H * W > 256)


def choose_conv_tile(N, H, W, taps, Ktot, Mpad, budget=LDS_LIMIT, out16=True, cus=256):
    padT, padB, padL, padR = _pads(taps)
    best = None
    for ltw in range(0, min(5, _pow2ceil_log(W)) + 1):
        for lth in range(0, min(8 - ltw, _pow2ceil_log(H)) + 1):
            for ltn in range(0, min(8 - ltw - lth, _pow2ceil_log(N)) + 1):
                TW, TH, TN = 1 << ltw, 1 << lth, 1 << ltn
                tiles = -(-W // TW) * -(-H // TH) * -(-N // TN)
                util = (N * H * W) / (tiles * 256.0)
                NP = TN * (TH + padT + padB) * (TW + padL + padR)
                mt1 = out16 and tiles <= cus and Mpad >= 64
                mt = 1 if mt1 else min(3, Mpad // 32)
                kcs = [kc for kc in ((16, 32, 48, 64, 96) if mt1 else (16, 32, 48, 64)) if Ktot % kc == 0]
                for kc in kcs:
                    lds = NP * (kc * 2 + 16) + 2 * mt * 32 * (kc * 2 + 16)
                    if len(taps) == 1 and Ktot // kc >= 2:
                        lds = max(lds, 2 * NP * kc * 2 + 2 * mt * 32 * (kc * 2 + 16))
                    if out16:
                        lds = max(lds, TN * TH * TW * (mt * 64 + 16) + mt * 128)
                    if lds > budget:
                        continue
                    allw = mt1 and len(taps) == 9 and NP * (kc * 2 + 16) + 9 * 32 * (kc * 2 + 16) <= LDS_LIMIT
                    flat = allw and TW == W and TH == H and TN * TH * TW == 256 and N % TN == 0 and kc <= 64
                    allw = (allw, flat)
                    halo = NP / float(TN * TH * TW)
                    key = (round(util, 3), mt1 or (lds <= CONV_LDS_PREFERRED and kc >= min(48, Ktot)), allw, kc, -round(halo, 3), ltw)
                    if best is None or key > best[0]:
                        best = (key, (ltw, lth, ltn, kc))
    if best is None:
        raise ValueError("no conv tiling fits in LDS for N=%d H=%d W=%d Ktot=%d" % (N, H, W, Ktot))
    return best[1]


def conv_fuses_pool(N, H, W, taps, Ktot, M, Mpad, ltw, lth, ltn, kc, cus):
    TW, TH, TN = 1 << ltw, 1 << lth, 1 << ltn
    padT, padB, padL, padR = _pads(taps)
    tiles = -(-W // TW) * -(-H // TH) * -(-N // TN)
    NP = TN * (TH + padT + padB) * (TW + padL + padR)
    m_last = M - (Mpad - 32)
    return (len(taps) == 9 and tiles <= cus and Mpad >= 64 and NP * (kc * 2 + 16) + 9 * 32 * (kc * 2 + 16) <= LDS_LIMIT and
            TW == W and TH == H and TN * TH * TW == 256 and N % TN == 0 and kc <= 64 and m_last in (32, 16, 8) and
            H % 2 == 0 and W % 2 == 0)


def _wg_stride(row_bytes):
    return ((row_bytes + 63) & ~127) + 64


def choose_wgrad_tile(N, H, W, taps, Kpad, Mpad, Ktot, M, cus, budget=LDS_LIMIT):
    padT, padB, padL, padR = _pads(taps)
    best = None
    for ltw in range(0, min(4, _pow2ceil_log(W)) + 1):
        for lth in range(0, min(8 - ltw, _pow2ceil_log(H)) + 1):
            for ltn in range(max(0, 5 - ltw - lth), 8 - ltw - lth + 1):
                if ltn > max(_pow2ceil_log(N), 5 - ltw - lth):
                    continue
                TW, TH, TN = 1 << ltw, 1 << lth, 1 << ltn
                tiles = -(-W // TW) * -(-H // TH) * -(-N // TN)
                util = (N * H * W) / float(tiles * TN * TH * TW)
                NP = TN * (TH + padT + padB) * (TW + padL + padR)
                HW_ = TW + padL + padR
                lds = 2 * ((NP + HW_) * _wg_stride(Kpad * 2) + (TN * TH * TW + TW) * _wg_stride(Mpad * 2)) + 4096
                if lds > budget:
                    continue
                HH, HW = TH + padT + padB, TW + padL + padR
                ix, idz = -(-(HW * (Ktot // 8)) // 64), -(-(TW * (M // 8)) // 64)
                rswx, rswd = -(-(TN * HH) // 4), -(-(TN * TH) // 4)
                steps = TN * TH * TW // 16 - 2
                single = tiles <= cus
                if idz > 3:
                    continue
                if not ((ix <= 4 and (single or rswx + rswd <= steps)) or
                        (ix <= 6 and (single or (rswx <= steps and rswd <= steps)))):
                    continue
                key = (round(util, 3), TN * TH * TW, -NP, ltw, -ltn)
                if best is None or key > best[0]:
                    best = (key, (ltw, lth, ltn), tiles)
    if best is None:
        raise ValueError("no wgrad tiling fits in LDS")
    return best[1], best[2]



class NetPlan:

    def __init__(self, prefix: str, in_channels: int, out_channels: int, blindspot: bool, B: int, H: int, W: int,
                 cus: int = 256, train: bool = True, param_base: int = 0, dev_cus: Optional[int] = None, input_grad: bool = False):
        if input_grad and not train:
            raise ValueError("input_grad needs a training plan (train=True)")
        if H % 32 or W % 32:
            raise ValueError("input height/width must be multiples of 32 (NoiseNetwork.input_wh_mul)")
        if blindspot and H != W:
            raise ValueError("blind-spot mode needs square inputs")
        self.prefix, self.C, self.Cout, self.blindspot = prefix, in_channels, out_channels, blindspot
        self.B, self.H, self.W, self.cus, self.train = B, H, W, cus, train
        self.input_grad = bool(input_grad)
        self.dev_cus = cus if dev_cus is None else dev_cus
        self.R = 4 if blindspot else 1
        self.N = self.R * B
        self.layers = net_layers(in_channels, out_channels, blindspot)
        self.nparams = net_param_count(self.layers)
        self.param_base = param_base
        self.taps3 = TAPS_BLIND if blindspot else TAPS_PLAIN
        self.tensors: Dict[str, TSpec] = {}
        self.fwd: List[Op] = []
        self.bwd: List[Op] = []
        self.pack: List[Op] = []
        self.max_slab = 0
        self.max_bslab = 0
        self._build()

    def T(self, name, kind, shape):
        full = self.prefix + name
        self.tensors[full] = TSpec(full, kind, tuple(int(s) for s in shape))
        return full

    def act(self, name, N, H, W, C):
        return self.T(name, "act", (N, H, W, C))

    def grad(self, name, N, H, W, C):
        return self.T(name, "actb", (N, H, W, C))

    def _conv(self, lst, layer: Layer, role: str, src0, c0, up0, src1, c1, N, H, W, taps, M, dst=None, dst32=None,
              bias=True, act=True, mask=None, add=None, pool=None, pool_shifted=0, upsum=None, upsum_mask=None, upsum_c=0,
              unrot=None, unrot_mask=None, unrot_smask=None, urot=None, urot_smask=None, sign_out=None, mask_sign=None, upsum_mask_sign=None):
        Ktot = c0 + c1
        Mpad = ceil_to(M, 32)
        if upsum is None:
            upsum_mask_sign = None
        ltw, lth, ltn, kc = choose_conv_tile(N, H, W, taps, Ktot, Mpad, out16=dst32 is None, cus=self.cus)
        fused = pool is not None and conv_fuses_pool(N, H, W, taps, Ktot, M, Mpad, ltw, lth, ltn, kc, self.dev_cus)
        if upsum is not None:
            dma = (len(taps) == 9 and H % 16 == 0 and W % 16 == 0 and cdma_fills(N * (H // 16) * (W // 16), self.dev_cus, H, W) and
                   Ktot % 48 in (0, 16) and upsum_c % 96 == 0)
            fused = (dma or conv_fuses_pool(N, H, W, taps, Ktot, M, Mpad, ltw, lth, ltn, kc, self.dev_cus)) and upsum_c % 8 == 0 and \
                mask is None and add is None
            if not fused:
                upsum = upsum_mask = None
            if not (fused and dma):
                upsum_mask_sign = None
        lst.append(Op("conv", dict(layer=layer.name, role=role, src0=src0, src1=src1, c0=c0, c1=c1, up0=int(up0), N=N, H=H, W=W,
                                   taps=list(taps), M=M, Mpad=Mpad, Ktot=Ktot, bias=bias, act=int(act), mask=mask, add=add,
                                   dst=dst, dst32=dst32, ltw=ltw, lth=lth, ltn=ltn, kc=kc, bf16=int(role == "dgrad"),
                                   kreal=(layer.cin if role == "fwd" else layer.M),
                                   pool=pool if (fused and pool is not None) else None,
                                   pool_shifted=int(pool_shifted) if (fused and pool is not None) else 0,
                                   upsum=upsum, upsum_mask=upsum_mask, upsum_c=int(upsum_c) if upsum is not None else 0,
                                   unrot=unrot, unrot_mask=unrot_mask, unrot_smask=unrot_smask,
                                   urot=urot, urot_smask=urot_smask, sign_out=sign_out, mask_sign=mask_sign,
                                   upsum_mask_sign=upsum_mask_sign)))
        return fused

    def _wgrad(self, layer: Layer, dz: View, Mz: int, src0, c0, up0, src1, c1, cin_real, N, H, W, taps,
               m_off=0, c_off=0, with_bias=True, cblocks=None, mblocks=1):
        Ktot = c0 + c1
        Kpad = ceil_to(Ktot, 32) if cblocks is None else 96
        coff = [0] * len(taps) if cblocks is None else list(cblocks)
        if cblocks is not None:
            taps = [(0, 0)] * len(cblocks)
        Mpad = ceil_to(Mz, 32)
        ntaps = len(taps)
        slab_bytes = ntaps * Mpad * Kpad * 4
        ctiles = ntaps * Kpad // 32 + 1
        if WGRAD_MEGA and self.cus >= 64 and self.N * self.H * self.W >= MEGA_MIN_PX:
            self.nwgrad = getattr(self, "nwgrad", 0) + 1
            op = Op("wgrad", dict(layer=layer.name, dz=dz, src0=src0, src1=src1, c0=c0, c1=c1, up0=int(up0), N=N, H=H, W=W,
                                  taps=list(taps), coff=coff, M=Mz, Mpad=Mpad, Ktot=Ktot, Kpad=Kpad, nslabs=0, ltw=0, lth=0, ltn=0,
# ... 386 lines not shown
```

selfsupervised-denoising_amd/ssdn/hip/lib.py:

```python
from __future__ import annotations

import ctypes as C
import os

_HERE = os.path.dirname(os.path.abspath(__file__))
LIB_PATH = os.environ.get("SSDN_HIP_LIB") or os.path.join(_HERE, "libssdn_hip.so")
MAX_TAPS = 9

OP = dict(pack_input=1, conv=2, pool_fwd=3, pool_bwd=4, upsum_bwd=5, unrot_fwd=6, unrot_bwd=7, wgrad=8, wreduce=9,
          wpack=10, grad_pack=11, head_ssdn=12, head_final=13, spatial_mean=14, mse=15, mask_mse=16, adam=17,
          metrics=18, zero=19, event_record=20, noise=21, input_grad=22, head_vjp=23,
          mse_vjp=24, accum=25)

i32, f32, vp = C.c_int32, C.c_float, C.c_void_p


class View(C.Structure):
    _fields_ = [("p", vp), ("cs", i32), ("co", i32)]


class OpRec(C.Structure):
    _fields_ = [("type", i32), ("lane", i32), ("args", vp)]


class PackInputArgs(C.Structure):
    _fields_ = [("src", vp), ("dst", View), ("B", i32), ("C", i32), ("H", i32), ("W", i32), ("R", i32), ("cpad", i32)]


class ConvArgs(C.Structure):
    _fields_ = [("src0", View), ("src1", View), ("c0", i32), ("c1", i32), ("up0", i32), ("N", i32), ("H", i32), ("W", i32),
                ("ntaps", i32), ("dy", i32 * MAX_TAPS), ("dx", i32 * MAX_TAPS), ("w", vp), ("M", i32), ("Mpad", i32),
                ("Ktot", i32), ("bias", vp), ("act", i32), ("mask", View), ("add", View), ("dst", View), ("dst32", vp),
                ("ltw", i32), ("lth", i32), ("ltn", i32), ("kc", i32), ("bf16", i32), ("wc", vp), ("kreal", i32),
                ("pool", View), ("pool_shifted", i32), ("upsum", View), ("upsum_mask", View), ("upsum_c", i32),
                ("unrot", View), ("unrot_mask", View), ("unrot_smask", vp),
                ("urot", View), ("urot_smask", vp), ("sign_out", vp), ("mask_sign", vp), ("upsum_mask_sign", vp)]


class PoolArgs(C.Structure):
    _fields_ = [("act", View), ("pooled", View), ("dpool", View), ("dz", View), ("N", i32), ("H", i32), ("W", i32),
                ("C", i32), ("shifted", i32), ("route", vp)]


class UpsumArgs(C.Structure):
    _fields_ = [("src", View), ("mask", View), ("dst", View), ("N", i32), ("H", i32), ("W", i32), ("C", i32)]


class UnrotArgs(C.Structure):
    _fields_ = [("src", View), ("dst", View), ("mask", View), ("B", i32), ("P", i32), ("C", i32), ("smask", vp)]


class WgradArgs(C.Structure):
    _fields_ = [("dz", View), ("src0", View), ("src1", View), ("c0", i32), ("c1", i32), ("up0", i32), ("N", i32),
                ("H", i32), ("W", i32), ("ntaps", i32), ("dy", i32 * MAX_TAPS), ("dx", i32 * MAX_TAPS), ("coff", i32 * MAX_TAPS),
                ("M", i32), ("Mpad", i32), ("Ktot", i32), ("Kpad", i32), ("slab", vp), ("bslab", vp), ("nslabs", i32), ("ltw", i32),
                ("lth", i32), ("ltn", i32), ("csplit", i32), ("mblocks", i32), ("kreal", i32), ("mega", i32), ("cost", C.c_float)]


class WreduceArgs(C.Structure):
    _fields_ = [("slab", vp), ("bslab", vp), ("nslabs", i32), ("ntaps", i32), ("M", i32), ("Mpad", i32), ("Kpad", i32),
                ("cin", i32), ("cin_full", i32), ("m_off", i32), ("c_off", i32), ("tapblock", i32), ("gw", vp), ("gb", vp),
                ("inv_scale", vp), ("accumulate", i32)]


class WpackArgs(C.Structure):
    _fields_ = [("w", vp), ("wf", vp), ("wd", vp), ("M", i32), ("cin", i32), ("ntaps", i32), ("c0", i32), ("c1_real", i32),
                ("Mpad_f", i32), ("Ktot", i32), ("Mpad_d", i32), ("Kd", i32), ("wfc", vp), ("wdc", vp)]


class GradPackArgs(C.Structure):
    _fields_ = [("g", vp), ("dst", View), ("N", i32), ("C", i32), ("H", i32), ("W", i32), ("cpad", i32), ("gmax", vp),
                ("scale_out", vp)]


class HeadArgs(C.Structure):
    _fields_ = [("net_out", vp), ("noisy", vp), ("noise_param", vp), ("est_raw", vp), ("B", i32), ("C", i32), ("H", i32),
                ("W", i32), ("style", i32), ("mode", i32), ("want_grad", i32), ("mu", vp), ("pme", vp), ("model_std", vp),
                ("noise_std", vp), ("g_net_out", vp), ("partial", vp), ("nchunks", i32), ("gmax", vp), ("diag", i32)]


class HeadFinalArgs(C.Structure):
    _fields_ = [("partial", vp), ("B", i32), ("nchunks", i32), ("H", i32), ("W", i32), ("mode", i32), ("loss", vp),
                ("g_est", vp), ("g_sigma_out", vp), ("gmax2", vp)]


class SpatialMeanArgs(C.Structure):
    _fields_ = [("src", vp), ("dst", vp), ("B", i32), ("HW", i32)]


class MseArgs(C.Structure):
    _fields_ = [("out", vp), ("ref", vp), ("coords", vp), ("ncoords", i32), ("B", i32), ("C", i32), ("H", i32), ("W", i32),
                ("loss", vp), ("g", vp), ("gmax", vp)]


class AdamArgs(C.Structure):
    _fields_ = [("p", vp), ("g", vp), ("m", vp), ("v", vp), ("n", C.c_int64), ("lr", f32), ("b1", f32), ("b2", f32),
                ("eps", f32), ("bc1", f32), ("bc2", f32), ("gscale", f32)]


class MetricsArgs(C.Structure):
    _fields_ = [("out", vp), ("mu", vp), ("clean", vp), ("loss", vp), ("model_std", vp), ("noise_std", vp), ("ext", vp),
                ("B", i32), ("C", i32), ("H", i32), ("W", i32), ("noise_n", i32), ("per", vp), ("acc", vp)]


class ZeroArgs(C.Structure):
    _fields_ = [("p", vp), ("bytes", C.c_int64)]


class EventArgs(C.Structure):
    _fields_ = [("event", vp)]


class NoiseArgs(C.Structure):
    _fields_ = [("clean_u8", vp), ("clean32", vp), ("noisy32", vp), ("ref32", vp), ("param", vp), ("param_ref", vp), ("coords", vp),
                ("B", i32), ("C", i32), ("H", i32), ("W", i32), ("style", i32), ("clip", i32), ("p_lo", f32), ("p_hi", f32),
                ("n2v_box", i32), ("n2v_radius", i32), ("seed", C.c_uint64), ("offset", C.c_uint64)]


class InputGradArgs(C.Structure):
    _fields_ = [("g_e0", View), ("g_d1a", View), ("w_e", vp), ("w_d", vp), ("out", vp), ("B", i32), ("C", i32), ("H", i32), ("W", i32),
                ("R", i32), ("ntaps", i32), ("dy", i32 * MAX_TAPS), ("dx", i32 * MAX_TAPS), ("add", vp)]


class HeadVjpArgs(C.Structure):
    _fields_ = [("net_out", vp), ("noisy", vp), ("noise_param", vp), ("est_raw", vp), ("B", i32), ("C", i32), ("H", i32), ("W", i32),
                ("style", i32), ("mode", i32), ("w", vp), ("g_pme", vp), ("g_mu", vp), ("keep", i32), ("nchunks", i32),
                ("g_net_out", vp), ("partial", vp), ("gmax", vp), ("g_est", vp), ("g_sigma_out", vp), ("gmax2", vp),
                ("g_noisy", vp), ("diag", i32)]


class MseVjpArgs(C.Structure):
    _fields_ = [("out", vp), ("ref", vp), ("coords", vp), ("ncoords", i32), ("masked", i32), ("B", i32), ("C", i32), ("H", i32),
                ("W", i32), ("keep", i32), ("w", vp), ("g_pme", vp), ("g", vp), ("gmax", vp)]


class AccumArgs(C.Structure):
    _fields_ = [("dst", vp), ("src", vp), ("n", C.c_int64)]


ARG_TYPES = dict(pack_input=PackInputArgs, conv=ConvArgs, pool_fwd=PoolArgs, pool_bwd=PoolArgs, upsum_bwd=UpsumArgs,
                 unrot_fwd=UnrotArgs, unrot_bwd=UnrotArgs, wgrad=WgradArgs, wreduce=WreduceArgs, wpack=WpackArgs,
                 grad_pack=GradPackArgs, head_ssdn=HeadArgs, head_final=HeadFinalArgs, spatial_mean=SpatialMeanArgs,
                 mse=MseArgs, mask_mse=MseArgs, adam=AdamArgs, metrics=MetricsArgs, zero=ZeroArgs, event_record=EventArgs, noise=NoiseArgs,
                 input_grad=InputGradArgs, head_vjp=HeadVjpArgs, mse_vjp=MseVjpArgs, accum=AccumArgs)

ABI_VERSION = 19

SYMBOLS = ["ssdn_run_ops", "ssdn_stream_order", "ssdn_conv_lds_bytes", "ssdn_wgrad_lds_bytes", "ssdn_abi_version", "ssdn_last_error",
           "ssdn_device_cus", "ssdn_probe_mfma", "ssdn_probe_tr16", "ssdn_struct_size", "ssdn_profile_enable",
           "ssdn_profile_read", "ssdn_profile_set_stride", "ssdn_debug_set_trace", "ssdn_debug_get_trace", "ssdn_conv_set_mode",
           "ssdn_wgrad_mergeable", "ssdn_conv_fuses_pool", "ssdn_conv_fuses_upsum", "ssdn_conv_fuses_unrot", "ssdn_conv_fuses_urot", "ssdn_conv_signs", "ssdn_chain_len",
           "ssdn_conv_set_chain", "ssdn_wgrad_mega_ok", "ssdn_wgrad_variant",
           "ssdn_plan_load", "ssdn_plan_destroy", "ssdn_plan_arena_bytes", "ssdn_plan_meta", "ssdn_plan_bind", "ssdn_plan_tensor", "ssdn_plan_run",
           "ssdn_plan_set_lr", "ssdn_net_forward", "ssdn_train_step"]
PLAN_PHASES = dict(repack=0, forward=1, backward=2, optimiser=3)
PROF = dict(conv_mt3=0, conv_mt2=1, conv_mt1=2, wgrad=3, gemm=4, cdma_mt3=5, cdma_mt21=6, wgrad_side=7)

def pointer_fields(st, base: int = 0):
    out = []
    for name, ty in st._fields_:
        off = base + getattr(st, name).offset
        if ty is vp:
            out.append(off)
        elif isinstance(ty, type) and issubclass(ty, C.Structure):
            out += pointer_fields(ty, off)
    return out


_lib = None


class SsdnHipError(RuntimeError):
    pass


def load() -> C.CDLL:
    global _lib
    if _lib is not None:
        return _lib
    if not os.path.exists(LIB_PATH):
        raise SsdnHipError("libssdn_hip.so not found at %s -- build it with `python -c 'import __graft_entry__ as g; g.build()'` "
                           "(the ssdn hot path has no CPU fallback)" % LIB_PATH)
    lib = C.CDLL(LIB_PATH)
    lib.ssdn_run_ops.argtypes = [C.POINTER(OpRec), C.c_int, vp]
    lib.ssdn_run_ops.restype = C.c_int
    if hasattr(lib, "ssdn_stream_order"):
        lib.ssdn_stream_order.argtypes = [vp, vp]
        lib.ssdn_stream_order.restype = C.c_int
    lib.ssdn_conv_lds_bytes.argtypes = [C.POINTER(ConvArgs)]
    lib.ssdn_conv_lds_bytes.restype = C.c_int
    lib.ssdn_wgrad_lds_bytes.argtypes = [C.POINTER(WgradArgs)]
    lib.ssdn_wgrad_lds_bytes.restype = C.c_int
    lib.ssdn_abi_version.restype = C.c_int
    lib.ssdn_last_error.restype = C.c_char_p
    lib.ssdn_device_cus.restype = C.c_int
    lib.ssdn_probe_mfma.argtypes = [vp, vp, vp, vp]
    lib.ssdn_probe_mfma.restype = C.c_int
    lib.ssdn_probe_tr16.argtypes = [vp, C.c_int, vp, vp, vp]
    lib.ssdn_probe_tr16.restype = C.c_int
    lib.ssdn_profile_enable.argtypes = [C.c_int, C.c_int]
    lib.ssdn_profile_enable.restype = C.c_int
    lib.ssdn_profile_set_stride.argtypes = [C.c_int, C.c_int]
    lib.ssdn_profile_set_stride.restype = C.c_int
    lib.ssdn_profile_read.argtypes = [C.c_int, C.POINTER(C.c_double), C.POINTER(C.c_longlong), C.POINTER(C.c_double), C.POINTER(C.c_double)]
    lib.ssdn_profile_read.restype = C.c_int
    lib.ssdn_conv_set_mode.argtypes = [C.c_int]
    lib.ssdn_conv_set_mode.restype = C.c_int
    lib.ssdn_conv_set_chain.argtypes = [C.c_int]
    lib.ssdn_conv_set_chain.restype = C.c_int
    lib.ssdn_chain_len.argtypes = [C.c_void_p, C.c_int]
    lib.ssdn_chain_len.restype = C.c_int
    lib.ssdn_conv_fuses_unrot.argtypes = [C.c_void_p]
    lib.ssdn_conv_fuses_unrot.restype = C.c_int
    lib.ssdn_conv_fuses_urot.argtypes = [C.c_void_p]
    lib.ssdn_conv_fuses_urot.restype = C.c_int
    lib.ssdn_conv_signs.argtypes = [C.c_void_p]
    lib.ssdn_conv_signs.restype = C.c_int
    lib.ssdn_conv_fuses_upsum.argtypes = [C.c_void_p]
    lib.ssdn_conv_fuses_upsum.restype = C.c_int
    lib.ssdn_conv_fuses_pool.argtypes = [C.c_void_p]
    lib.ssdn_conv_fuses_pool.restype = C.c_int
    lib.ssdn_wgrad_mergeable.argtypes = [C.c_void_p]
    lib.ssdn_wgrad_mergeable.restype = C.c_int
    lib.ssdn_wgrad_mega_ok.argtypes = [C.c_void_p]
    lib.ssdn_wgrad_mega_ok.restype = C.c_int
    lib.ssdn_wgrad_variant.argtypes = [C.c_void_p, C.POINTER(C.c_int32)]
    lib.ssdn_wgrad_variant.restype = C.c_int
    lib.ssdn_struct_size.argtypes = [C.c_int]
    lib.ssdn_struct_size.restype = C.c_int
    lib.ssdn_plan_load.argtypes = [C.c_void_p, C.c_int64, C.POINTER(C.c_void_p)]
    lib.ssdn_plan_load.restype = C.c_int
    lib.ssdn_plan_destroy.argtypes = [C.c_void_p]
    lib.ssdn_plan_destroy.restype = None
    lib.ssdn_plan_arena_bytes.argtypes = [C.c_void_p]
    lib.ssdn_plan_arena_bytes.restype = C.c_int64
    lib.ssdn_plan_meta.argtypes = [C.c_void_p]
    lib.ssdn_plan_meta.restype = C.c_char_p
    lib.ssdn_plan_bind.argtypes = [C.c_void_p, C.c_void_p]
    lib.ssdn_plan_bind.restype = C.c_int
    lib.ssdn_plan_tensor.argtypes = [C.c_void_p, C.c_char_p, C.POINTER(C.c_void_p), C.POINTER(C.c_int64)]
    lib.ssdn_plan_tensor.restype = C.c_int
    lib.ssdn_plan_run.argtypes = [C.c_void_p, C.c_int, C.c_void_p]
    lib.ssdn_plan_run.restype = C.c_int
    lib.ssdn_plan_set_lr.argtypes = [C.c_void_p, C.c_float, C.c_int, C.c_float]
    lib.ssdn_plan_set_lr.restype = C.c_int
    lib.ssdn_net_forward.argtypes = [C.c_void_p, C.c_void_p]
    lib.ssdn_net_forward.restype = C.c_int
    lib.ssdn_train_step.argtypes = [C.c_void_p, C.c_float, C.c_int, C.c_void_p]
    lib.ssdn_train_step.restype = C.c_int
    if lib.ssdn_abi_version() != ABI_VERSION:
        raise SsdnHipError("libssdn_hip.so ABI version mismatch")
    if os.environ.get("SSDN_CHAIN_MODE"):
        lib.ssdn_conv_set_chain(int(os.environ["SSDN_CHAIN_MODE"]))
    _lib = lib
    return lib


def check(rc: int):
    if rc != 0:
        raise SsdnHipError(load().ssdn_last_error().decode())
```

Baseline: 21900.

## Fuse SSDN loss head, head-final reduction and first backward grad-pack/dgrad conv

Adds a head_junction op and kernel that computes the per-pixel SSDN head loss and gradient, then in the same kernel packs the gradient and applies the first backward 1x1 dgrad conv via MFMA. A ticket/terms scheme finishes the cross-block loss reduction in the same kernel. The backward pass skips the now-redundant grad_pack/conv ops when the junction has run. This removes several launches and the round trip of the fp32 head gradient through global memory. In exchange it adds grid-wide atomic ticket synchronisation and fp-contract-controlled FMAs to keep the numerics matched.

```diff
diff --git a/include/ssdn_hip.h b/include/ssdn_hip.h
--- a/include/ssdn_hip.h
+++ b/include/ssdn_hip.h
@@ -44,7 +44,8 @@
     SSDN_OP_INPUT_GRAD = 22,
     SSDN_OP_HEAD_VJP = 23,
     SSDN_OP_MSE_VJP = 24,
-    SSDN_OP_ACCUM = 25
+    SSDN_OP_ACCUM = 25,
+    SSDN_OP_HEAD_JUNCTION = 26
 };
 
 typedef struct ssdn_op {
@@ -207,6 +208,15 @@
     uint32_t* gmax2;
 } ssdn_head_final_args;
 
+typedef struct ssdn_head_junction_args {
+    ssdn_head_args head;
+    ssdn_head_final_args fin;
+    ssdn_grad_pack_args gp;
+    ssdn_conv_args conv;
+    float* terms;
+    uint32_t* tickets;
+} ssdn_head_junction_args;
+
 typedef struct ssdn_spatial_mean_args {
     const float* src;
     float* dst;
diff --git a/selfsupervised-denoising_amd/csrc/api.hip b/selfsupervised-denoising_amd/csrc/api.hip
--- a/selfsupervised-denoising_amd/csrc/api.hip
+++ b/selfsupervised-denoising_amd/csrc/api.hip
@@ -103,6 +103,7 @@
         case SSDN_OP_HEAD_VJP: return (int)sizeof(ssdn_head_vjp_args);
         case SSDN_OP_MSE_VJP: return (int)sizeof(ssdn_mse_vjp_args);
         case SSDN_OP_ACCUM: return (int)sizeof(ssdn_accum_args);
+        case SSDN_OP_HEAD_JUNCTION: return (int)sizeof(ssdn_head_junction_args);
         default: return -1;
     }
 }
@@ -335,6 +336,7 @@
             }
             case SSDN_OP_HEAD_SSDN: rc = launch_head((const ssdn_head_args*)p, s); break;
             case SSDN_OP_HEAD_FINAL: rc = launch_head_final((const ssdn_head_final_args*)p, s); break;
+            case SSDN_OP_HEAD_JUNCTION: rc = launch_head_junction((const ssdn_head_junction_args*)p, s); break;
             case SSDN_OP_SPATIAL_MEAN: rc = launch_spatial_mean((const ssdn_spatial_mean_args*)p, s); break;
             case SSDN_OP_MSE: rc = launch_mse((const ssdn_mse_args*)p, 0, s); break;
             case SSDN_OP_MASK_MSE: rc = launch_mse((const ssdn_mse_args*)p, 1, s); break;
diff --git a/selfsupervised-denoising_amd/csrc/common.h b/selfsupervised-denoising_amd/csrc/common.h
--- a/selfsupervised-denoising_amd/csrc/common.h
+++ b/selfsupervised-denoising_amd/csrc/common.h
@@ -128,6 +128,7 @@
 int launch_head(const ssdn_head_args* a, hipStream_t s);
 int launch_head_impulse(const ssdn_head_args* a, hipStream_t s);
 int launch_head_final(const ssdn_head_final_args* a, hipStream_t s);
+int launch_head_junction(const ssdn_head_junction_args* a, hipStream_t s);
 int launch_spatial_mean(const ssdn_spatial_mean_args* a, hipStream_t s);
 int launch_mse(const ssdn_mse_args* a, int masked, hipStream_t s);
 int launch_head_vjp(const ssdn_head_vjp_args* a, hipStream_t s);
diff --git a/selfsupervised-denoising_amd/csrc/head.hip b/selfsupervised-denoising_amd/csrc/head.hip
--- a/selfsupervised-denoising_amd/csrc/head.hip
+++ b/selfsupervised-denoising_amd/csrc/head.hip
@@ -25,7 +25,7 @@
 }
 
 template <bool DIAG>
-__global__ void k_head(ssdn_head_args a) {
+__global__ __launch_bounds__(HB) void k_head(ssdn_head_args a) {
     __shared__ float sh[4];
     const int b = blockIdx.y;
     const long long HW = (long long)a.H * a.W;
@@ -127,88 +127,10 @@
                 gest_acc += dsig * dsig_dest;
             }
         } else {
-            float mu[3], A[6], y[3], sig[3], dsig_dmu[3], dsig_dest[3];
-#pragma unroll
-            for (int c = 0; c < 3; ++c) { mu[c] = no[c * HW + p]; y[c] = ny[c * HW + p]; }
-#pragma unroll
-            for (int c = 0; c < 6; ++c) A[c] = no[(3 + c) * HW + p];
-#pragma unroll
-            for (int c = 0; c < 3; ++c) {
-                if (a.style == 0) {
-                    sig[c] = a.mode == 0 ? fmaxf(npar, 1e-3f) : est;
-                    dsig_dmu[c] = 0.f;
-                    dsig_dest[c] = 1.f;
-                } else {
-                    float m = fmaxf(mu[c], 1e-3f);
-                    float f = a.mode == 0 ? 1.f / npar : est;
-                    sig[c] = sqrtf(m * f);
-                    dsig_dmu[c] = mu[c] > 1e-3f ? 0.5f * f / sig[c] : 0.f;
-                    dsig_dest[c] = 0.5f * m / sig[c];
-                }
-            }
-            float x00 = A[0] * A[0] + A[1] * A[1] + A[2] * A[2];
-            float x01 = A[1] * A[3] + A[2] * A[4];
-            float x02 = A[2] * A[5];
-            float x11 = A[3] * A[3] + A[4] * A[4];
-            float x12 = A[4] * A[5];
-            float x22 = A[5] * A[5];
-            float n0 = sig[0] * sig[0], n1 = sig[1] * sig[1], n2 = sig[2] * sig[2];
-            float s00 = x00 + n0, s01 = x01, s02 = x02, s11 = x11 + n1, s12 = x12, s22 = x22 + n2;
-            float c00 = s11 * s22 - s12 * s12, c01 = s02 * s12 - s01 * s22, c02 = s01 * s12 - s02 * s11;
-            float c11 = s00 * s22 - s02 * s02, c12 = s01 * s02 - s00 * s12, c22 = s00 * s11 - s01 * s01;
-            float det = s00 * c00 + s01 * c01 + s02 * c02;
-            float rdet = 1.f / det;
-            float i00 = c00 * rdet, i01 = c01 * rdet, i02 = c02 * rdet, i11 = c11 * rdet, i12 = c12 * rdet, i22 = c22 * rdet;
-            float d0 = y[0] - mu[0], d1 = y[1] - mu[1], d2 = y[2] - mu[2];
-            float q0 = i00 * d0 + i01 * d1 + i02 * d2;
-            float q1 = i01 * d0 + i11 * d1 + i12 * d2;
-            float q2 = i02 * d0 + i12 * d1 + i22 * d2;
-            float quad = d0 * q0 + d1 * q1 + d2 * q2;
-            float detc = fmaxf(det, 0.f);
-            float l = 0.5f * logf(detc) + 0.5f * quad;
-            if (a.mode != 0) l -= 0.1f * (sig[0] + sig[1] + sig[2]) * (1.f / 3.f);
+            float l, gs = 0.f, gv[9];
+            head_pixel_full3(a, no, ny, b, p, HW, npar, est, inv_total, true, l, gs, gv, gabs);
             loss_acc += l;
-            long long o3 = (long long)b * 3 * HW + p;
-            if (a.mu) { a.mu[o3] = mu[0]; a.mu[o3 + HW] = mu[1]; a.mu[o3 + 2 * HW] = mu[2]; }
-            if (a.pme) {
-                const float e = 1e-6f;
-                float t00 = s00 + 2 * e, t11 = s11 + 2 * e, t22 = s22 + 2 * e;
-                float k00 = t11 * t22 - s12 * s12, k01 = s02 * s12 - s01 * t22, k02 = s01 * s12 - s02 * t11;
-                float k11 = t00 * t22 - s02 * s02, k12 = s01 * s02 - t00 * s12, k22 = t00 * t11 - s01 * s01;
-                float rd = 1.f / (t00 * k00 + s01 * k01 + s02 * k02);
-                float r0 = (k00 * d0 + k01 * d1 + k02 * d2) * rd;
-                float r1 = (k01 * d0 + k11 * d1 + k12 * d2) * rd;
-                float r2 = (k02 * d0 + k12 * d1 + k22 * d2) * rd;
-                a.pme[o3] = mu[0] + (x00 + e) * r0 + x01 * r1 + x02 * r2;
-                a.pme[o3 + HW] = mu[1] + x01 * r0 + (x11 + e) * r1 + x12 * r2;
-                a.pme[o3 + 2 * HW] = mu[2] + x02 * r0 + x12 * r1 + (x22 + e) * r2;
-            }
-            if (a.model_std) a.model_std[(long long)b * HW + p] = cbrtf(fabsf(A[0] * A[3] * A[5]));
-            if (a.noise_std && a.style == 1) a.noise_std[(long long)b * HW + p] = cbrtf(sig[0] * sig[1] * sig[2]);
-            if (a.want_grad) {
-                float hd = det > 0.f ? 0.5f : 0.f;
-                float g00 = hd * i00 - 0.5f * q0 * q0, g01 = hd * i01 - 0.5f * q0 * q1, g02 = hd * i02 - 0.5f * q0 * q2;
-                float g11 = hd * i11 - 0.5f * q1 * q1, g12 = hd * i12 - 0.5f * q1 * q2, g22 = hd * i22 - 0.5f * q2 * q2;
-                float reg = a.mode != 0 ? 0.1f / 3.f : 0.f;
-                float ds0 = 2.f * sig[0] * g00 - reg, ds1 = 2.f * sig[1] * g11 - reg, ds2 = 2.f * sig[2] * g22 - reg;
-                float g[9];
-                g[0] = -q0 + ds0 * dsig_dmu[0];
-                g[1] = -q1 + ds1 * dsig_dmu[1];
-                g[2] = -q2 + ds2 * dsig_dmu[2];
-                g[3] = 2.f * (g00 * A[0]);
-                g[4] = 2.f * (g00 * A[1] + g01 * A[3]);
-                g[5] = 2.f * (g00 * A[2] + g01 * A[4] + g02 * A[5]);
-                g[6] = 2.f * (g01 * A[1] + g11 * A[3]);
-                g[7] = 2.f * (g01 * A[2] + g11 * A[4] + g12 * A[5]);
-                g[8] = 2.f * (g02 * A[2] + g12 * A[4] + g22 * A[5]);
-#pragma unroll
-                for (int c = 0; c < 9; ++c) {
-                    float v = g[c] * inv_total;
-                    a.g_net_out[((long long)b * 9 + c) * HW + p] = v;
-                    gabs = fmaxf(gabs, fabsf(v));
-                }
-                gest_acc += ds0 * dsig_dest[0] + ds1 * dsig_dest[1] + ds2 * dsig_dest[2];
-            }
+            if (a.want_grad) gest_acc += gs;
         }
     }
     float ls = block_sum(loss_acc, sh);
diff --git a/selfsupervised-denoising_amd/csrc/head_common.h b/selfsupervised-denoising_amd/csrc/head_common.h
--- a/selfsupervised-denoising_amd/csrc/head_common.h
+++ b/selfsupervised-denoising_amd/csrc/head_common.h
@@ -38,3 +38,93 @@
     float x = raw - 4.f;
     return x > 20.f ? 1.f : 1.f / (1.f + expf(-x));
 }
+
+static __device__ __forceinline__ float hfma(float a, float b, float c) { return __builtin_fmaf(a, b, c); }
+static __device__ __forceinline__ void head_pixel_full3(const ssdn_head_args& a, const float* no, const float* ny, int b, long long p, long long HW,
+                                                        float npar, float est, float inv_total, bool st, float& l_out, float& gs_out,
+                                                        float (&gv)[9], float& gabs) {
+#pragma clang fp contract(off)
+    float mu[3], A[6], y[3], sig[3], dsig_dmu[3], dsig_dest[3];
+#pragma unroll
+    for (int c = 0; c < 3; ++c) { mu[c] = no[c * HW + p]; y[c] = ny[c * HW + p]; }
+#pragma unroll
+    for (int c = 0; c < 6; ++c) A[c] = no[(3 + c) * HW + p];
+#pragma unroll
+    for (int c = 0; c < 3; ++c) {
+        if (a.style == 0) {
+            sig[c] = a.mode == 0 ? fmaxf(npar, 1e-3f) : est;
+            dsig_dmu[c] = 0.f;
+            dsig_dest[c] = 1.f;
+        } else {
+            float m = fmaxf(mu[c], 1e-3f);
+            float f = a.mode == 0 ? 1.f / npar : est;
+            sig[c] = sqrtf(m * f);
+            dsig_dmu[c] = mu[c] > 1e-3f ? 0.5f * f / sig[c] : 0.f;
+            dsig_dest[c] = 0.5f * m / sig[c];
+        }
+    }
+    float x00 = hfma(A[2], A[2], hfma(A[1], A[1], A[0] * A[0]));
+    float x01 = hfma(A[2], A[4], A[1] * A[3]);
+    float x02 = A[2] * A[5];
+    float x11 = hfma(A[4], A[4], A[3] * A[3]);
+    float x12 = A[4] * A[5];
+    float x22 = A[5] * A[5];
+    float n0 = sig[0] * sig[0], n1 = sig[1] * sig[1], n2 = sig[2] * sig[2];
+    float s00 = x00 + n0, s01 = x01, s02 = x02, s11 = x11 + n1, s12 = x12, s22 = x22 + n2;
+    float c00 = hfma(s11, s22, -(s12 * s12)), c01 = hfma(s02, s12, -(s01 * s22)), c02 = hfma(s01, s12, -(s02 * s11));
+    float c11 = hfma(s00, s22, -(s02 * s02)), c12 = hfma(s01, s02, -(s00 * s12)), c22 = hfma(s00, s11, -(s01 * s01));
+    float det = hfma(s02, c02, hfma(s01, c01, s00 * c00));
+    float rdet = 1.f / det;
+    float i00 = c00 * rdet, i01 = c01 * rdet, i02 = c02 * rdet, i11 = c11 * rdet, i12 = c12 * rdet, i22 = c22 * rdet;
+    float d0 = y[0] - mu[0], d1 = y[1] - mu[1], d2 = y[2] - mu[2];
+    float q0 = hfma(i02, d2, hfma(i01, d1, i00 * d0));
+    float q1 = hfma(i12, d2, hfma(i11, d1, i01 * d0));
+    float q2 = hfma(i22, d2, hfma(i12, d1, i02 * d0));
+    float quad = hfma(d2, q2, hfma(d1, q1, d0 * q0));
+    float detc = fmaxf(det, 0.f);
+    float l = hfma(0.5f, quad, 0.5f * logf(detc));
+    if (a.mode != 0) l -= 0.1f * (sig[0] + sig[1] + sig[2]) * (1.f / 3.f);
+    l_out = l;
+    long long o3 = (long long)b * 3 * HW + p;
+    if (st && a.mu) { a.mu[o3] = mu[0]; a.mu[o3 + HW] = mu[1]; a.mu[o3 + 2 * HW] = mu[2]; }
+    if (st && a.pme) {
+        const float e = 1e-6f;
+        float t00 = s00 + 2 * e, t11 = s11 + 2 * e, t22 = s22 + 2 * e;
+        float k00 = hfma(t11, t22, -(s12 * s12)), k01 = hfma(s02, s12, -(s01 * t22)), k02 = hfma(s01, s12, -(s02 * t11));
+        float k11 = hfma(t00, t22, -(s02 * s02)), k12 = hfma(s01, s02, -(t00 * s12)), k22 = hfma(t00, t11, -(s01 * s01));
+        float rd = 1.f / hfma(s02, k02, hfma(s01, k01, t00 * k00));
+        float r0 = hfma(k02, d2, hfma(k01, d1, k00 * d0)) * rd;
+        float r1 = hfma(k12, d2, hfma(k11, d1, k01 * d0)) * rd;
+        float r2 = hfma(k22, d2, hfma(k12, d1, k02 * d0)) * rd;
+        a.pme[o3] = hfma(x02, r2, hfma(x01, r1, hfma(x00 + e, r0, mu[0])));
+        a.pme[o3 + HW] = hfma(x12, r2, hfma(x11 + e, r1, hfma(x01, r0, mu[1])));
+        a.pme[o3 + 2 * HW] = hfma(x22 + e, r2, hfma(x12, r1, hfma(x02, r0, mu[2])));
+    }
+    if (st && a.model_std) a.model_std[(long long)b * HW + p] = cbrtf(fabsf(A[0] * A[3] * A[5]));
+    if (st && a.noise_std && a.style == 1) a.noise_std[(long long)b * HW + p] = cbrtf(sig[0] * sig[1] * sig[2]);
+    if (a.want_grad) {
+        float hd = det > 0.f ? 0.5f : 0.f;
+        float g00 = hfma(hd, i00, -(0.5f * q0 * q0)), g01 = hfma(hd, i01, -(0.5f * q0 * q1)), g02 = hfma(hd, i02, -(0.5f * q0 * q2));
+        float g11 = hfma(hd, i11, -(0.5f * q1 * q1)), g12 = hfma(hd, i12, -(0.5f * q1 * q2)), g22 = hfma(hd, i22, -(0.5f * q2 * q2));
+        float reg = a.mode != 0 ? 0.1f / 3.f : 0.f;
+        float ds0 = hfma(2.f * sig[0], g00, -reg), ds1 = hfma(2.f * sig[1], g11, -reg), ds2 = hfma(2.f * sig[2], g22, -reg);
+        float g[9];
+        g[0] = hfma(ds0, dsig_dmu[0], -q0);
+        g[1] = hfma(ds1, dsig_dmu[1], -q1);
+        g[2] = hfma(ds2, dsig_dmu[2], -q2);
+        g[3] = 2.f * (g00 * A[0]);
+        g[4] = 2.f * hfma(g01, A[3], g00 * A[1]);
+        g[5] = 2.f * hfma(g02, A[5], hfma(g01, A[4], g00 * A[2]));
+        g[6] = 2.f * hfma(g11, A[3], g01 * A[1]);
+        g[7] = 2.f * hfma(g12, A[5], hfma(g11, A[4], g01 * A[2]));
+        g[8] = 2.f * hfma(g22, A[5], hfma(g12, A[4], g02 * A[2]));
+#pragma unroll
+        for (int c = 0; c < 9; ++c) {
+            float v = g[c] * inv_total;
+            if (st) a.g_net_out[((long long)b * 9 + c) * HW + p] = v;
+            gv[c] = v;
+            gabs = fmaxf(gabs, fabsf(v));
+        }
+        gs_out = hfma(ds2, dsig_dest[2], hfma(ds1, dsig_dest[1], ds0 * dsig_dest[0]));
+    }
+}
diff --git a/selfsupervised-denoising_amd/csrc/head_junction.hip b/selfsupervised-denoising_amd/csrc/head_junction.hip
--- /dev/null
+++ b/selfsupervised-denoising_amd/csrc/head_junction.hip
@@ -0,0 +1,206 @@
+#include "head_common.h"
+#include <cstdlib>
+
+#define JN_THREADS HB
+#ifndef JN_TILES
+#define JN_TILES 2
+#endif
+#define JN_WG_PX (4 * JN_TILES * 32)
+#define JN_OSTR (96 * 2 + 16)
+#define JN_SMEM (4 * 32 * JN_OSTR)
+#define JN_MAX_PARTIALS (JN_SMEM / 8)
+
+struct jn_args {
+    ssdn_head_args h;
+    const h16* w;
+    ssdn_view gz, mask, dst;
+    float* scale_out;
+    float* loss;
+    float* g_est;
+    float* terms;
+    uint32_t* tickets;
+    int nsub;
+    int ablate;
+};
+#ifdef SSDN_TUNING
+#define JN_ABLATE(j, bit) ((j).ablate & (bit))
+#else
+#define JN_ABLATE(j, bit) 0
+#endif
+
+static __device__ __forceinline__ void jn_publish2(float* p, float x, float y) {
+    const unsigned long long v = (unsigned long long)__float_as_uint(x) | ((unsigned long long)__float_as_uint(y) << 32);
+    __hip_atomic_store(reinterpret_cast<unsigned long long*>(p), v, __ATOMIC_RELAXED, __HIP_MEMORY_SCOPE_AGENT);
+}
+static __device__ __forceinline__ void jn_fetch2(const float* p, float& x, float& y) {
+    const unsigned long long v = __hip_atomic_load(reinterpret_cast<const unsigned long long*>(p), __ATOMIC_RELAXED, __HIP_MEMORY_SCOPE_AGENT);
+    x = __uint_as_float((unsigned)v);
+    y = __uint_as_float((unsigned)(v >> 32));
+}
+
+__global__ __launch_bounds__(JN_THREADS) void k_head_junction(jn_args j) {
+    __shared__ __attribute__((aligned(16))) char smem[JN_SMEM];
+    __shared__ float sh[4];
+    __shared__ int last;
+    const ssdn_head_args& a = j.h;
+    const int tid = threadIdx.x, lane = tid & 63, l31 = lane & 31, kh = lane >> 5;
+    const int wave = tid >> 6;
+    char* reg = smem + wave * (32 * JN_OSTR);
+    const int HW = a.H * a.W;
+    const int sub = blockIdx.x % j.nsub, bc = blockIdx.x / j.nsub;
+    const int chunk = bc % a.nchunks, b = bc / a.nchunks;
+    const float inv_total = 1.f / ((float)a.B * (float)HW);
+    float est = 0.f, dest_draw = 0.f;
+    if (a.mode != 0) {
+        float raw = a.est_raw[0];
+        est = softplus_m4(raw);
+        dest_draw = sigmoid_m4(raw);
+    }
+    const float npar = a.noise_param ? a.noise_param[b] : 0.f;
+    const int per = (HW + a.nchunks - 1) / a.nchunks;
+    const int p0 = chunk * per;
+    const int p1 = p0 + per < HW ? p0 + per : HW;
+    const float* no = a.net_out + (long long)b * 9 * HW;
+    const float* ny = a.noisy + (long long)b * 3 * HW;
+    if (blockIdx.x == 0 && tid == 0 && j.scale_out) { j.scale_out[0] = 1.f; j.scale_out[1] = 1.f; }
+    half8 af[3];
+#pragma unroll
+    for (int mt = 0; mt < 3; ++mt) af[mt] = *reinterpret_cast<const half8*>(j.w + (mt * 32 + l31) * 16 + kh * 8);
+    float gabs = 0.f;
+    for (int ti = 0; ti < JN_TILES; ++ti) {
+        const int t0 = p0 + sub * JN_WG_PX + (ti * 4 + wave) * 32;
+        if (t0 >= p1) break;
+        const int p = t0 + l31;
+        const long long pix0 = (long long)b * HW + t0;
+        u32x4_t mk[6];
+#pragma unroll
+        for (int u = 0; u < 6; ++u) {
+            const int e = lane + 64 * u, px = e / 12, cc = e - px * 12;
+            mk[u] = *reinterpret_cast<const u32x4_t*>((const h16*)j.mask.p + j.mask.co + (pix0 + px) * j.mask.cs + cc * 8);
+        }
+        float l, gs = 0.f, gv[9];
+        head_pixel_full3(a, no, ny, b, p, HW, npar, est, inv_total, kh == 0 && !JN_ABLATE(j, 2), l, gs, gv, gabs);
+        if (kh == 0) jn_publish2(j.terms + (pix0 + l31) * 2, l, gs);
+        u16x8 gz = zero_b8();
+        if (kh == 0) {
+#pragma unroll
+            for (int c = 0; c < 8; ++c) gz[c] = f2bf(gv[c]);
+        } else gz[0] = f2bf(gv[8]);
+        st_b8((unsigned short*)j.gz.p + j.gz.co + (pix0 + l31) * j.gz.cs + kh * 8, gz);
+        if (JN_ABLATE(j, 1)) continue;
+        f32x16 zero;
+#pragma unroll
+        for (int r = 0; r < 16; ++r) zero[r] = 0.f;
+#pragma unroll
+        for (int mt = 0; mt < 3; ++mt) {
+            const f32x16 acc = __builtin_amdgcn_mfma_f32_32x32x16_bf16(__builtin_bit_cast(bf16x8, af[mt]), __builtin_bit_cast(bf16x8, gz), zero, 0, 0, 0);
+#pragma unroll
+            for (int g = 0; g < 4; ++g) {
+                u32x2_t o;
+                o[0] = pack_bf16x2(acc[g * 4 + 0], acc[g * 4 + 1]);
+                o[1] = pack_bf16x2(acc[g * 4 + 2], acc[g * 4 + 3]);
+                *reinterpret_cast<u32x2_t*>(reg + l31 * JN_OSTR + (mt * 32 + g * 8 + kh * 4) * 2) = o;
+            }
+        }
+        asm volatile("s_waitcnt lgkmcnt(0)" ::: "memory");
+        __builtin_amdgcn_wave_barrier();
+#pragma unroll
+        for (int u = 0; u < 6; ++u) {
+            const int e = lane + 64 * u, px = e / 12, cc = e - px * 12;
+            u32x4_t o = *reinterpret_cast<const u32x4_t*>(reg + px * JN_OSTR + cc * 16);
+#pragma unroll
+            for (int w = 0; w < 4; ++w) {
+                const float v0 = bf_lo(o[w]) * lrelu_grad(f16_lo(mk[u][w]));
+                const float v1 = bf_hi(o[w]) * lrelu_grad(f16_hi(mk[u][w]));
+                o[w] = pack_bf16x2(v0, v1);
+            }
+            *reinterpret_cast<u32x4_t*>((h16*)j.dst.p + j.dst.co + (pix0 + px) * j.dst.cs + cc * 8) = o;
+        }
+        asm volatile("s_waitcnt lgkmcnt(0)" ::: "memory");
+        __builtin_amdgcn_wave_barrier();
+    }
+    if (a.gmax) atomic_max_abs_block(a.gmax, gabs, sh);
+    if (sub == 0 && chunk == 0 && tid == 0 && a.noise_std && a.style == 0) a.noise_std[b] = a.mode == 0 ? fmaxf(npar, 1e-3f) : est;
+    if (JN_ABLATE(j, 4)) return;
+    asm volatile("s_waitcnt vmcnt(0)" ::: "memory");
+    __syncthreads();
+    if (tid == 0) last = __hip_atomic_fetch_add(j.tickets + 1 + bc, 1u, __ATOMIC_RELAXED, __HIP_MEMORY_SCOPE_AGENT) == (unsigned)j.nsub - 1;
+    __syncthreads();
+    if (!last) return;
+    float loss_acc = 0.f, gest_acc = 0.f;
+    const float* tb = j.terms + (long long)b * HW * 2;
+    for (int pb = p0 + tid; pb < p1; pb += 8 * HB) {
+        float tl[8], tg[8];
+#pragma unroll
+        for (int u = 0; u < 8; ++u) {
+            tl[u] = tg[u] = 0.f;
+            if (pb + u * HB < p1) jn_fetch2(tb + 2 * (pb + u * HB), tl[u], tg[u]);
+        }
+#pragma unroll
+        for (int u = 0; u < 8; ++u)
+            if (pb + u * HB < p1) { loss_acc += tl[u]; gest_acc += tg[u]; }
+    }
+    const float ls = block_sum(loss_acc, sh);
+    const float gs = block_sum(gest_acc, sh);
+    const int nparts = a.B * a.nchunks;
+    if (tid == 0) {
+        jn_publish2(a.partial + (long long)bc * 2, ls, gs * dest_draw * inv_total);
+        __hip_atomic_store(j.tickets + 1 + bc, 0u, __ATOMIC_RELAXED, __HIP_MEMORY_SCOPE_AGENT);
+        asm volatile("s_waitcnt vmcnt(0)" ::: "memory");
+        last = __hip_atomic_fetch_add(j.tickets, 1u, __ATOMIC_RELAXED, __HIP_MEMORY_SCOPE_AGENT) == (unsigned)nparts - 1;
+    }
+    __syncthreads();
+    if (!last) return;
+    float* st = reinterpret_cast<float*>(smem);
+    for (int i = tid; i < nparts; i += HB) jn_fetch2(a.partial + 2 * i, st[2 * i], st[2 * i + 1]);
+    __syncthreads();
+    for (int bb = tid; bb < a.B; bb += HB) {
+        float l = 0.f;
+        for (int c = 0; c < a.nchunks; ++c) l += st[(bb * a.nchunks + c) * 2];
+        j.loss[bb] = l / (float)HW;
+    }
+    if (a.mode == 1 && j.g_est && tid == 0) {
+        float g = 0.f;
+        for (int bb = 0; bb < a.B; ++bb)
+            for (int c = 0; c < a.nchunks; ++c) g += st[(bb * a.nchunks + c) * 2 + 1];
+        j.g_est[0] = g;
+    }
+    if (tid == 0) __hip_atomic_store(j.tickets, 0u, __ATOMIC_RELAXED, __HIP_MEMORY_SCOPE_AGENT);
+}
+
+int launch_head_junction(const ssdn_head_junction_args* q, hipStream_t s) {
+    const ssdn_head_args& h = q->head;
+    const ssdn_head_final_args& f = q->fin;
+    if (h.C != 3 || h.diag || h.style < 0 || h.style > 1 || h.mode < 0 || h.mode > 1 || !h.want_grad)
+        return ssdn_set_error("head_junction: serves C = 3, full covariance, style gauss / poisson, mode known / const, want_grad = 1");
+    if (h.B < 1 || h.H < 1 || h.W < 1 || h.nchunks < 1) return ssdn_set_error("head_junction: bad shape");
+    if (!h.net_out || !h.noisy || !h.g_net_out || !h.partial || !f.loss || !q->terms || !q->tickets)
+        return ssdn_set_error("head_junction: net_out, noisy, g_net_out, partial, loss, terms and tickets must be given");
+    if (h.mode == 0 && !h.noise_param) return ssdn_set_error("head_junction: mode known needs noise_param");
+    if (h.mode != 0 && !h.est_raw) return ssdn_set_error("head_junction: mode const needs est_raw");
+    if (f.partial != h.partial || f.B != h.B || f.nchunks != h.nchunks || f.H != h.H || f.W != h.W || f.mode != h.mode)
+        return ssdn_set_error("head_junction: the reduction does not belong to the head");
+    const long long HW = (long long)h.H * h.W, per = (HW + h.nchunks - 1) / h.nchunks;
+    if (HW % 32 || per % 32) return ssdn_set_error("head_junction: H*W and the chunk length must be multiples of 32");
+    if ((long long)h.B * h.nchunks > JN_MAX_PARTIALS) return ssdn_set_error("head_junction: more than %d partials", JN_MAX_PARTIALS);
+    if (q->gp.g != h.g_net_out || q->gp.C != 9 || q->gp.N != h.B || q->gp.H != h.H || q->gp.W != h.W)
+        return ssdn_set_error("head_junction: the gradient pack does not read the head's g_net_out");
+    if (!conv_gradpack_fusable(&q->gp, &q->conv)) return ssdn_set_error("head_junction: the data gradient cannot ride behind the gradient pack");
+    jn_args j;
+    j.h = h;
+    j.w = (const h16*)q->conv.w;
+    j.gz = q->gp.dst; j.mask = q->conv.mask; j.dst = q->conv.dst;
+    j.scale_out = q->gp.scale_out;
+    j.loss = f.loss;
+    j.g_est = f.g_est;
+    j.terms = q->terms;
+    j.tickets = q->tickets;
+    j.nsub = (int)((per + JN_WG_PX - 1) / JN_WG_PX);
+    static const int env_ablate = [] { const char* e = ssdn_tuning_env("SSDN_JN_ABLATE"); return e ? atoi(e) : 0; }();
+    j.ablate = env_ablate;
+    const long long grid = (long long)h.B * h.nchunks * j.nsub;
+    if (grid >= (1ll << 31)) return ssdn_set_error("head_junction: grid too large");
+    SSDN_LAUNCH(k_head_junction, dim3((unsigned)grid), dim3(JN_THREADS), 0, s, j);
+    SSDN_CHECK_HIP(hipGetLastError());
+    return 0;
+}
diff --git a/selfsupervised-denoising_amd/ssdn/hip/engine.py b/selfsupervised-denoising_amd/ssdn/hip/engine.py
--- a/selfsupervised-denoising_amd/ssdn/hip/engine.py
+++ b/selfsupervised-denoising_amd/ssdn/hip/engine.py
@@ -74,6 +74,21 @@
         self.bwd_head = OpList(self._bwd_recs[:len(self._bwd_recs) - len(self.tail_recs)], lanes=True) if self.tail_recs else None
         self.pack = OpList([self._mat(op) for op in plan.pack])
         self.accumulate = False
+        self.bwd_skip = self.bwd_head_skip = None
+
+    def junction_pair(self):
+        r = self._bwd_recs
+        if len(r) < 3 or r[0][0] != "grad_pack" or r[1][0] != "conv" or any(len(x) > 2 and x[2] != 0 for x in r[:2]):
+            return None
+        gp, cv = r[0][1], r[1][1]
+        if cv.ntaps != 1 or cv.Ktot != 16 or cv.M != 96 or not cv.bf16 or not cv.mask.p or cv.src0.p != gp.dst.p or gp.C != 9:
+            return None
+        return gp, cv
+
+    def make_skip_lists(self):
+        self.bwd_skip = OpList(self._bwd_recs[2:], lanes=True)
+        if self.bwd_head is not None:
+            self.bwd_head_skip = OpList(self._bwd_recs[2:len(self._bwd_recs) - len(self.tail_recs)], lanes=True)
 
     def set_accumulate(self, on: bool) -> None:
         self.accumulate = bool(on)
@@ -403,6 +418,13 @@
 MODE = {"known": 0, "const": 1, "var": 2}
 
 
+def junction_served(pipeline: str, C: int, diag: bool, style: str, mode: str, B: int, H: int, W: int, nchunks: int) -> bool:
+    HW = H * W
+    per = (HW + nchunks - 1) // nchunks
+    return (pipeline == "ssdn" and C == 3 and not diag and style in ("gauss", "poisson") and mode in ("known", "const") and
+            HW % 32 == 0 and per % 32 == 0 and B * nchunks <= 3328)
+
+
 def engine_style(style: str) -> str:
     return "poisson" if style.startswith("poisson") else "impulse" if style.startswith("impulse") else "gauss"
 
@@ -463,6 +485,13 @@
         self.g_est_stage = torch.zeros((1,), **f32) if self.stages_est else None
         self._head_final_args = None
         self._accum_ops = None
+        self.junction = self._junction_ok()
+        self.junction_fresh = False
+        self._junction_args = None
+        if self.junction:
+            self.head_terms = torch.zeros((B, H * W, 2), **f32)
+            self.head_tickets = torch.zeros((1 + B * self.nchunks,), dtype=torch.int32, device=device)
+            self.main.make_skip_lists()
         self.metrics_per = torch.zeros((B, 8), **f32)
         self._metrics_args = None
         self.ops_loss = OpList(self._loss_ops(want_grad=train))
@@ -473,6 +502,11 @@
         self.gen = 0
         self.g_fresh = self.loss_fwd = False
         self._vjp = None
+
+    def _junction_ok(self) -> bool:
+        from . import graph as G
+        return bool(G.HEAD_JUNCTION and self.train and self.main.junction_pair() is not None and
+                    junction_served(self.pipeline, self.C, self.diag, self.style, self.mode, self.B, self.H, self.W, self.nchunks))
 
     def _gmax(self, net: Optional[DeviceNet]):
         if net is not None and self.train:
@@ -491,15 +525,24 @@
                 est_ptr = _ptr(self.est_raw)
             elif self.mode == "const":
                 est_ptr = _ptr(self.params, 4 * self.est_off)
-            recs.append(("head_ssdn", L.HeadArgs(_ptr(out32), _ptr(self.inp), _ptr(self.noise_param), est_ptr, B, Cn, H, W,
-                                                  STYLE[self.style], MODE[self.mode], int(want_grad), _ptr(self.mu), _ptr(self.pme),
-                                                  _ptr(self.model_std), _ptr(self.noise_std), g32, _ptr(self.partial),
-                                                  self.nchunks, self._gmax(self.main), int(self.diag))))
+            head = L.HeadArgs(_ptr(out32), _ptr(self.inp), _ptr(self.noise_param), est_ptr, B, Cn, H, W,
+                              STYLE[self.style], MODE[self.mode], int(want_grad), _ptr(self.mu), _ptr(self.pme),
+                              _ptr(self.model_std), _ptr(self.noise_std), g32, _ptr(self.partial),
+                              self.nchunks, self._gmax(self.main), int(self.diag))
             g_est = self._g_est_ptr() if want_grad else None
-            recs.append(("head_final", L.HeadFinalArgs(_ptr(self.partial), B, self.nchunks, H, W, MODE[self.mode], _ptr(self.loss), g_est,
-                                                        _ptr(self.sigma.tensor("g32")) if (want_grad and self.sigma is not None) else None,
-                                                        self._gmax(self.sigma) if self.sigma is not None else None)))
-            self._head_final_args = recs[-1][1]
+            final = L.HeadFinalArgs(_ptr(self.partial), B, self.nchunks, H, W, MODE[self.mode], _ptr(self.loss), g_est,
+                                    _ptr(self.sigma.tensor("g32")) if (want_grad and self.sigma is not None) else None,
+                                    self._gmax(self.sigma) if self.sigma is not None else None)
+            if self.junction and want_grad:
+                j = self._junction_args = L.HeadJunctionArgs()
+                j.head, j.fin = head, final
+                j.gp, j.conv = self.main.junction_pair()
+                j.terms, j.tickets = _ptr(self.head_terms), _ptr(self.head_tickets)
+                recs.append(("head_junction", j))
+                self._head_final_args = j.fin
+            else:
+                recs += [("head_ssdn", head), ("head_final", final)]
+                self._head_final_args = final
         elif self.pipeline == "mse":
             recs.append(("mse", L.MseArgs(_ptr(out32), _ptr(self.ref), None, 0, B, Cn, H, W, _ptr(self.loss), g32, self._gmax(self.main))))
         elif self.pipeline == "mask_mse":
@@ -588,6 +631,8 @@
                  ("noise_param", self.noise_param), ("coords", self.coords), ("partial", self.partial), ("est_raw", self.est_raw),
                  ("g_est_var", self.g_est_var), ("mu", self.mu), ("pme", self.pme), ("model_std", self.model_std), ("noise_std", self.noise_std),
                  ("zero_buf", self.zero_buf), ("metrics_per", self.metrics_per)]
+        if self.junction:
+            tens += [("head_terms", self.head_terms), ("head_tickets", self.head_tickets)]
         tens = [(n, t) for n, t in tens if t is not None]
         table, by_ptr = [], {}
         for name, t in tens:
@@ -631,7 +676,7 @@
         train = self.train
         phases = [[self.main.pack, self.sigma.pack if self.sigma is not None else None],
                   [self.main.fwd, self.sigma.fwd if self.sigma is not None else None, self.ops_loss],
-                  [self.main.bwd, self.sigma.bwd if self.sigma is not None else None] if train else [],
+                  [self.main.bwd_skip if self.junction else self.main.bwd, self.sigma.bwd if self.sigma is not None else None] if train else [],
                   [self.ops_opt] if train else []]
         layers = lambda net, base: [dict(name=l.name, w_off=base + l.w_off, b_off=base + l.b_off, M=l.M, cin=l.cin, k=l.k) for l in net.plan.layers]
         desc = dict(pipeline=self.pipeline, channels=self.C, blindspot=bool(self.blindspot), style=self.style, mode=self.mode, diag=self.diag, B=self.B, H=self.H,
@@ -682,12 +727,14 @@
             if self.sigma is not None:
                 self.sigma.fwd.run(s)
         self.ops_loss.run(s)
+        self.junction_fresh = self.junction and self.train
 
     def net_forward_only(self, stream=None):
         s = current_stream() if stream is None else stream
         if self.train:
             self.gen += 1
             self.g_fresh = self.loss_fwd = False
+        self.junction_fresh = False
         self.main.fwd.run(s)
 
     def _head_addend(self, on: bool) -> None:
@@ -699,15 +746,19 @@
     def backward(self, stream=None, exchange=None, defer_tail=False, with_head_dx=False):
         s = current_stream() if stream is None else stream
         self._head_addend(with_head_dx)
+        skip = self.junction_fresh and self.g_fresh
+        self.junction_fresh = False
+        bwd = self.main.bwd_skip if skip else self.main.bwd
+        bwd_head = self.main.bwd_head_skip if skip else self.main.bwd_head
         if self.accumulate and self.stages_est:
             self._accum_ops.run(s)
         if defer_tail and exchange is None and self.ops_opt_tail is not None:
             if self.sigma is not None and (int(self.SIGMA_CONCURRENT) & 2):
                 ev = self._fork_sigma(s, self.sigma.bwd)
-                self.main.bwd_head.run(s)
+                bwd_head.run(s)
                 self._join_sigma(s, ev)
             else:
-                self.main.bwd_head.run(s)
+                bwd_head.run(s)
                 if self.sigma is not None:
                     self.sigma.bwd.run(s)
             self._held_input_grad(s)
@@ -735,10 +786,10 @@
             return
         if self.sigma is not None and (int(self.SIGMA_CONCURRENT) & 2):
             ev = self._fork_sigma(s, self.sigma.bwd)
-            self.main.bwd.run(s)
+            bwd.run(s)
             self._join_sigma(s, ev)
         else:
-            self.main.bwd.run(s)
+            bwd.run(s)
             if self.sigma is not None:
                 self.sigma.bwd.run(s)
         self._held_input_grad(s)
diff --git a/selfsupervised-denoising_amd/ssdn/hip/graph.py b/selfsupervised-denoising_amd/ssdn/hip/graph.py
--- a/selfsupervised-denoising_amd/ssdn/hip/graph.py
+++ b/selfsupervised-denoising_amd/ssdn/hip/graph.py
@@ -11,6 +11,7 @@
 MID_WGRAD_PX, MID_WGRAD_G = 131072, 2
 WGRAD_CU_FRAC = (3, 4)
 WGRAD_MEGA = "split"
+HEAD_JUNCTION = True
 FUSE_UNROT_FWD = True
 SIGN_BYTES_HEAD = True
 X16_SLOTS = 16
diff --git a/selfsupervised-denoising_amd/ssdn/hip/lib.py b/selfsupervised-denoising_amd/ssdn/hip/lib.py
--- a/selfsupervised-denoising_amd/ssdn/hip/lib.py
+++ b/selfsupervised-denoising_amd/ssdn/hip/lib.py
@@ -10,7 +10,7 @@
 OP = dict(pack_input=1, conv=2, pool_fwd=3, pool_bwd=4, upsum_bwd=5, unrot_fwd=6, unrot_bwd=7, wgrad=8, wreduce=9,
           wpack=10, grad_pack=11, head_ssdn=12, head_final=13, spatial_mean=14, mse=15, mask_mse=16, adam=17,
           metrics=18, zero=19, event_record=20, noise=21, input_grad=22, head_vjp=23,
-          mse_vjp=24, accum=25)
+          mse_vjp=24, accum=25, head_junction=26)
 
 i32, f32, vp = C.c_int32, C.c_float, C.c_void_p
 
@@ -138,11 +138,15 @@
     _fields_ = [("dst", vp), ("src", vp), ("n", C.c_int64)]
 
 
+class HeadJunctionArgs(C.Structure):
+    _fields_ = [("head", HeadArgs), ("fin", HeadFinalArgs), ("gp", GradPackArgs), ("conv", ConvArgs), ("terms", vp), ("tickets", vp)]
+
+
 ARG_TYPES = dict(pack_input=PackInputArgs, conv=ConvArgs, pool_fwd=PoolArgs, pool_bwd=PoolArgs, upsum_bwd=UpsumArgs,
                  unrot_fwd=UnrotArgs, unrot_bwd=UnrotArgs, wgrad=WgradArgs, wreduce=WreduceArgs, wpack=WpackArgs,
                  grad_pack=GradPackArgs, head_ssdn=HeadArgs, head_final=HeadFinalArgs, spatial_mean=SpatialMeanArgs,
                  mse=MseArgs, mask_mse=MseArgs, adam=AdamArgs, metrics=MetricsArgs, zero=ZeroArgs, event_record=EventArgs, noise=NoiseArgs,
-                 input_grad=InputGradArgs, head_vjp=HeadVjpArgs, mse_vjp=MseVjpArgs, accum=AccumArgs)
+                 input_grad=InputGradArgs, head_vjp=HeadVjpArgs, mse_vjp=MseVjpArgs, accum=AccumArgs, head_junction=HeadJunctionArgs)
 
 ABI_VERSION = 19
 
```

Result: no change. 22090 (median of 6 runs) (+0.9%).
